# andompesta/nodeembedding-to-communityembedding

Hardware: AMD Instinct MI355X
Metric: SGNS pair-updates/sec at d=128, 1M-node graph (higher is better)
Workload: dtype f32

## Files before the change

### include/come.h

```cpp
#ifndef COME_H_
#define COME_H_

#include <stdint.h>

#ifdef __cplusplus
extern "C" {
#endif

#define COME_ABI_VERSION 5

enum {
    COME_OK = 0,
    COME_E_INVALID = -1,
    COME_E_HIP = -2,
    COME_E_UNSUPPORTED = -3
};

enum {
    COME_MODE_HOGWILD = 0,
    COME_MODE_SEQUENTIAL = 1
};

#define COME_TABLE_PACKED 0x100

#define COME_HOT_NONE 0x200

#define COME_DEFAULT_HOT_SHARE 5e-6
#define COME_DEFAULT_HOT_SHARE_WIDE 8e-7

int come_abi_version(void);

const char *come_source_sha256(void);
const char *come_last_error(void);

int come_init(int device);

void come_exp_table(float *out1000);

int come_fast_version(void);

int come_sgns_o2(float *node, float *ctx, int64_t V, int d, const int32_t *walks, int64_t P,
                 int L, const uint64_t *seeds, int window, int negative, const uint32_t *table,
                 uint64_t T, float lr, float alpha, int mode, void *stream);

int come_pack_table(const uint32_t *table, uint64_t T, void *packed, int32_t *status,
                    void *stream);

int come_sgns_o1(float *node, int64_t V, int d, const int32_t *edges, int64_t E,
                 const uint64_t *seeds, int negative, const uint32_t *table, uint64_t T, float lr,
                 int mode, void *stream);

int come_sgns_o2_loss(const float *node, const float *ctx, int64_t V, int d, const int32_t *walks,
                      int64_t P, int L, const uint64_t *seeds, int window, int negative,
                      const uint32_t *table, uint64_t T, int flags, double *walk_out,
                      double *loss_out, int64_t *pairs_out, void *stream);
int come_sgns_pairs_loss(const float *inp, const float *out, int64_t V, int d,
                         const int32_t *rows_in, const int32_t *rows_pos, const int32_t *rows_neg,
                         int64_t M, int negative, double *pair_out, double *loss_out,
                         int64_t *pairs_out, void *stream);

int come_community_grad(float *x, int64_t V, int d, const float *pi, const float *mu,
                        const float *inv_cov, int K, float beta, float lr, int iters,
                        void *stream);

int come_community_loss(const float *x, int64_t V, int d, const float *pi, const float *prec_chol,
                        const float *mu_prec, const float *log_norm, int K, float *row_out,
                        double *loss_out, void *stream);

int come_gmm_resp(const float *x, int64_t V, int d, const float *prec_chol, const float *mu_prec,
                  const float *log_norm, int K, float *resp_out, void *stream);

int come_gmm_estep(const float *x, int64_t V, int d, const float *prec_chol, const float *mu_prec,
                   const float *log_norm, int K, float *resp_out, float *lse_out, void *stream);

int come_gmm_scatter(const float *x, int64_t V, int d, const float *resp, const float *means,
                     int K, int chunks, float *scratch, float *scatter_out, void *stream);

int come_gmm_params(const double *scatter, const double *nk, const double *means,
                    const double *weights, int K, int d, double reg_covar, double *cov_out,
                    double *prec_chol_out, float *e_prec_chol, float *e_mu_prec,
                    float *e_log_norm, int *info, void *stream);

int come_gmm_estep_diag(const float *x, int64_t V, int d, const float *prec_sqrt,
                        const float *mu_prec, const float *log_norm, int K, float *resp_out,
                        float *lse_out, void *stream);
int come_gmm_diag_scratch(int64_t V, int d, int K, int cus, int *chunks_out,
                          int *rows_per_chunk_out);
int come_gmm_diag_moments(const float *x, int64_t V, int d, const float *resp, int K, int chunks,
                          void *scratch, double *nk_out, double *sx_out, void *stream);
int come_gmm_diag_scatter(const float *x, int64_t V, int d, const float *resp, const float *means,
                          int K, int chunks, void *scratch, double *ssq_out, void *stream);
int come_community_grad_diag(float *x, int64_t V, int d, const float *pi, const float *mu,
                             const float *inv_var, int K, float beta, float lr, int iters,
                             void *stream);
int come_community_loss_diag(const float *x, int64_t V, int d, const float *pi,
                             const float *prec_sqrt, const float *mu_prec, const float *log_norm,
                             int K, float *row_out, double *loss_out, void *stream);

int come_kmeans_scratch(int64_t V, int d, int K, int cus, int *chunks_out,
                        int *rows_per_chunk_out);
int come_kmeans_lloyd(const float *x, int64_t V, int d, const float *centers, int K, int chunks,
                      void *scratch, int32_t *labels_out, float *mindist_out, double *sums_out,
                      int64_t *counts_out, double *inertia_out, void *stream);
int come_kmeans_assign(const float *x, int64_t V, int d, const float *centers, int K,
                       int32_t *labels_out, float *mindist_out, void *stream);
int come_kmeans_update(float *centers, const double *sums, const int64_t *counts, int K, int d,
                       double *stats2, void *stream);

int come_kmeans_pp_scratch(int64_t V, int d, int T, int cus, int *chunks_out,
                           int *rows_per_chunk_out);
int come_kmeans_pp_step(const float *x, int64_t V, int d, const float *closest,
                        const int32_t *cand, int T, int chunks, float *dist_out, double *ppot,
                        double *pots_out, void *stream);
int come_kmeans_pp_pick(const float *dist, int64_t V, int T, const double *ppot,
                        const double *pots, int chunks, float *closest_out, double *cpot_out,
                        int32_t *best_out, double *pot_out, void *stream);
int come_kmeans_pp_sample(const float *closest, int64_t V, const double *cpot, int chunks,
                          int rows_per_chunk, const double *u, int T, int32_t *cand_out,
                          void *stream);


int come_random_walks(const int64_t *rowptr, const int32_t *col, int64_t V,
                      const int32_t *starts, int64_t P, int path_length, float alpha,
                      uint64_t seed, int64_t walk_offset, const int32_t *emit, int32_t *out,
                      void *stream);

int come_walks_reference(const int64_t *rowptr, const int32_t *col, int64_t V, int n_streams,
                         const int32_t *paths_per_stream, uint32_t *states, int path_length,
                         double alpha, const int32_t *emit, int threads, int32_t *out);

int come_pyrandom_seed(uint64_t seed, uint32_t *state625);

int come_pyrandom_draw(uint32_t *state625, int kind, uint64_t arg, int64_t count, double *out);

int come_np_draw_seeds(uint32_t *state625, int64_t n, uint64_t *out);

int come_graph_from_edges(const int64_t *edges, int64_t E, int64_t *node_ids, int64_t *V_out,
                          int64_t *rowptr, int32_t *col, int64_t *degree, int32_t *edge_pos,
                          int64_t *E_out);

int come_read_int_rows(const char *path, int64_t *rows, int64_t cap_rows, int width,
                       int64_t *nrows_out, int *max_tokens_out);
int come_write_int_rows(const char *path, const int64_t *rows, int64_t nrows, int width,
                        int append);
int come_save_embedding(const char *path, const float *emb, int64_t V, int d, int64_t first_id);
int come_format_f32(float x, char *out32);

int come_delta_begin(const float *W, const float *S, float *D, float *Down, int64_t n,
                     void *stream);
int come_delta_end(float *W, float *S, const float *Dsum, const float *Down, int64_t n,
                   void *stream);

int come_delta_flags(const float *W, const float *S, int64_t rows, int d, uint8_t *flags,
                     void *stream);
int come_delta_gather(const float *W, const float *S, const int64_t *idx, int64_t n, int d,
                      float *D, float *Down, void *stream);
int come_delta_scatter(float *W, float *S, const int64_t *idx, int64_t n, int d,
                       const float *Dsum, const float *Down, void *stream);

typedef struct come_launch_opts {
    int o2_kernel;
    int o2_blocks_per_cu;
    int o2_waves_per_block;
    int o2_static;
    int rows_per_wave;
    int o1_rows_per_wave;
    int max_waves;
    int o1_blocks_per_cu;
    int resident_cap;
    int community_async;
    int gmm_cov_async;
    int walk_staged;
    int o2_fresh_loads;
    int o2_atomic_writeback;
    int gmm_resp16;
    int o1_chunk;
    uint64_t *o2_update_count;
} come_launch_opts;

int come_get_options(come_launch_opts *out);

int come_set_option(const char *name, int value);

int come_sgns_o2_ex(float *node, float *ctx, int64_t V, int d, const int32_t *walks, int64_t P,
                    int L, const uint64_t *seeds, int window, int negative,
                    const uint32_t *table, uint64_t T, float lr, float alpha, int mode,
                    const uint32_t *hot_rows, const come_launch_opts *opts, void *stream);

int come_hot_rows(const uint32_t *table, uint64_t T, int64_t V, uint64_t min_count,
                  uint32_t *counts, uint32_t *hot_bits, void *stream);
int come_sgns_o1_ex(float *node, int64_t V, int d, const int32_t *edges, int64_t E,
                    const uint64_t *seeds, int negative, const uint32_t *table, uint64_t T,
                    float lr, int mode, const uint32_t *hot_rows, const come_launch_opts *opts,
                    void *stream);

int come_cpu_sgns_o2(float *node, float *ctx, int64_t V, int d, const int32_t *walks, int64_t P,
                     int L, const uint64_t *seeds, int window, int negative, const uint32_t *table,
                     uint64_t T, float lr, float alpha, int mode, int threads, int64_t *pairs_out);
int come_cpu_sgns_o1(float *node, int64_t V, int d, const int32_t *edges, int64_t E,
                     const uint64_t *seeds, int negative, const uint32_t *table, uint64_t T,
                     float lr, int mode, int threads, int64_t *pairs_out);
int come_cpu_community_grad(float *x, int64_t V, int d, const float *pi, const float *mu,
                            const float *inv_cov, int K, float beta, float lr, int iters,
                            int threads);
int come_cpu_gmm_resp(const float *x, int64_t V, int d, const float *prec_chol,
                      const float *mu_prec, const float *log_norm, int K, float *resp_out,
                      int threads);
int come_cpu_gmm_estep(const float *x, int64_t V, int d, const float *prec_chol,
                       const float *mu_prec, const float *log_norm, int K, float *resp_out,
                       float *lse_out, int threads);
int come_cpu_community_loss(const float *x, int64_t V, int d, const float *pi,
                            const float *prec_chol, const float *mu_prec, const float *log_norm,
                            int K, float *row_out, double *loss_out, int threads);
int come_cpu_sgns_o2_loss(const float *node, const float *ctx, int64_t V, int d,
                          const int32_t *walks, int64_t P, int L, const uint64_t *seeds,
                          int window, int negative, const uint32_t *table, uint64_t T,
                          double *walk_out, double *loss_out, int64_t *pairs_out, int threads);
int come_cpu_sgns_pairs_loss(const float *inp, const float *out, int64_t V, int d,
                             const int32_t *rows_in, const int32_t *rows_pos,
                             const int32_t *rows_neg, int64_t M, int negative, double *pair_out,
                             double *loss_out, int64_t *pairs_out, int threads);


int come_make_table(const double *counts_by_id, int64_t V, uint32_t *table, uint64_t T,
                    double power);

int come_lcg_table_draws(uint64_t seed, int64_t count, const uint32_t *table, uint64_t T,
                         uint32_t *out);

int64_t come_count_o2_pairs(const int32_t *walks, int64_t P, int L, int window);

#ifdef __cplusplus
}
#endif

#endif
```

### nodeembedding-to-communityembedding_amd/_lib.py

```python
import contextlib
import ctypes
import os

HERE = os.path.dirname(os.path.abspath(__file__))
DEFAULT_LIB_PATH = os.path.join(HERE, "libcome.so")
LIB_PATH = os.environ.get("COME_LIB_PATH") or DEFAULT_LIB_PATH

MODE_HOGWILD = 0
MODE_SEQUENTIAL = 1
TABLE_PACKED = 0x100
HOT_NONE = 0x200
ABI_VERSION = 5

SYMBOLS = ("come_abi_version", "come_last_error", "come_init", "come_exp_table",
           "come_fast_version", "come_sgns_o2", "come_sgns_o1", "come_community_grad",
           "come_gmm_resp", "come_make_table", "come_count_o2_pairs", "come_set_option",
           "come_random_walks", "come_walks_reference", "come_pyrandom_seed",
           "come_pyrandom_draw", "come_np_draw_seeds", "come_graph_from_edges",
           "come_read_int_rows",
           "come_write_int_rows", "come_save_embedding", "come_format_f32",
           "come_gmm_estep", "come_gmm_scatter", "come_gmm_params", "come_pack_table",
           "come_delta_begin", "come_delta_end", "come_get_options", "come_sgns_o2_ex",
           "come_sgns_o1_ex", "come_hot_rows", "come_lcg_table_draws", "come_delta_flags",
           "come_delta_gather", "come_delta_scatter", "come_cpu_sgns_o2", "come_cpu_sgns_o1",
           "come_cpu_community_grad", "come_cpu_gmm_resp", "come_cpu_gmm_estep",
           "come_source_sha256", "come_kmeans_scratch", "come_kmeans_lloyd",
           "come_kmeans_assign", "come_kmeans_update", "come_kmeans_pp_scratch",
           "come_kmeans_pp_step", "come_kmeans_pp_pick", "come_kmeans_pp_sample",
           "come_community_loss", "come_cpu_community_loss", "come_sgns_o2_loss",
           "come_sgns_pairs_loss", "come_cpu_sgns_o2_loss", "come_cpu_sgns_pairs_loss",
           "come_gmm_estep_diag", "come_gmm_diag_scratch", "come_gmm_diag_moments",
           "come_gmm_diag_scatter", "come_community_grad_diag", "come_community_loss_diag")

OPTION_FIELDS = ("o2_kernel", "o2_blocks_per_cu", "o2_waves_per_block",
                 "o2_static", "rows_per_wave", "o1_rows_per_wave",
                 "max_waves", "o1_blocks_per_cu", "resident_cap", "community_async",
                 "gmm_cov_async", "walk_staged", "o2_fresh_loads", "o2_atomic_writeback",
                 "gmm_resp16", "o1_chunk")


class LaunchOpts(ctypes.Structure):
    _fields_ = [(f, ctypes.c_int) for f in OPTION_FIELDS] + [("o2_update_count",
                                                             ctypes.c_void_p)]

_lib = None


def source_sha256():
    import hashlib
    csrc = os.path.join(HERE, "csrc")
    header = os.path.join(os.path.dirname(HERE), "include", "come.h")
    if not os.path.isdir(csrc) or not os.path.exists(header):
        return None
    names = sorted(f for f in os.listdir(csrc) if f.endswith((".hip", ".cpp", ".h")))
    h = hashlib.sha256()
    for f in [os.path.join(csrc, n) for n in names] + [os.path.join(csrc, "Makefile"), header]:
        with open(f, "rb") as fh:
            h.update(fh.read())
    return h.hexdigest()


class ComeError(RuntimeError):
    pass


def build():
    import subprocess
    subprocess.check_call(["make", "-s", "-C", os.path.join(HERE, "csrc"), "-j4"])


def lib():
    global _lib
    if _lib is not None:
        return _lib
    if not os.path.exists(LIB_PATH):
        raise ComeError("libcome.so not found at %s -- build it with "
                        "`make -C nodeembedding-to-communityembedding_amd/csrc` or "
                        "`python -c 'import __graft_entry__ as g; g.build()'`" % LIB_PATH)
    import torch
    L = ctypes.CDLL(LIB_PATH)
    P, i32, i64, u64, f32, f64 = (ctypes.c_void_p, ctypes.c_int, ctypes.c_int64, ctypes.c_uint64,
                                  ctypes.c_float, ctypes.c_double)
    L.come_abi_version.restype = i32
    L.come_source_sha256.restype = ctypes.c_char_p
    L.come_last_error.restype = ctypes.c_char_p
    L.come_init.argtypes = [i32]
    L.come_exp_table.argtypes = [P]
    L.come_exp_table.restype = None
    L.come_sgns_o2.argtypes = [P, P, i64, i32, P, i64, i32, P, i32, i32, P, u64, f32, f32, i32, P]
    L.come_sgns_o1.argtypes = [P, i64, i32, P, i64, P, i32, P, u64, f32, i32, P]
    L.come_community_grad.argtypes = [P, i64, i32, P, P, P, i32, f32, f32, i32, P]
    L.come_community_loss.argtypes = [P, i64, i32, P, P, P, P, i32, P, P, P]
    L.come_gmm_resp.argtypes = [P, i64, i32, P, P, P, i32, P, P]
    L.come_pack_table.argtypes = [P, u64, P, P, P]
    L.come_delta_begin.argtypes = [P, P, P, P, i64, P]
    L.come_delta_end.argtypes = [P, P, P, P, i64, P]
    L.come_gmm_estep.argtypes = [P, i64, i32, P, P, P, i32, P, P, P]
    L.come_gmm_scatter.argtypes = [P, i64, i32, P, P, i32, i32, P, P, P]
    L.come_gmm_params.argtypes = [P, P, P, P, i32, i32, f64, P, P, P, P, P, P, P]
    L.come_gmm_estep_diag.argtypes = [P, i64, i32, P, P, P, i32, P, P, P]
    L.come_gmm_diag_scratch.argtypes = [i64, i32, i32, i32, P, P]
    L.come_gmm_diag_moments.argtypes = [P, i64, i32, P, i32, i32, P, P, P, P]
    L.come_gmm_diag_scatter.argtypes = [P, i64, i32, P, P, i32, i32, P, P, P]
    L.come_community_grad_diag.argtypes = [P, i64, i32, P, P, P, i32, f32, f32, i32, P]
    L.come_community_loss_diag.argtypes = [P, i64, i32, P, P, P, P, i32, P, P, P]
    L.come_kmeans_scratch.argtypes = [i64, i32, i32, i32, P, P]
    L.come_kmeans_lloyd.argtypes = [P, i64, i32, P, i32, i32, P, P, P, P, P, P, P]
    L.come_kmeans_assign.argtypes = [P, i64, i32, P, i32, P, P, P]
    L.come_kmeans_update.argtypes = [P, P, P, i32, i32, P, P]
    L.come_kmeans_pp_scratch.argtypes = [i64, i32, i32, i32, P, P]
    L.come_kmeans_pp_step.argtypes = [P, i64, i32, P, P, i32, i32, P, P, P, P]
    L.come_kmeans_pp_pick.argtypes = [P, i64, i32, P, P, i32, P, P, P, P, P]
    L.come_kmeans_pp_sample.argtypes = [P, i64, P, i32, i32, P, i32, P, P]
    L.come_make_table.argtypes = [P, i64, P, u64, f64]
    L.come_count_o2_pairs.argtypes = [P, i64, i32, i32]
    L.come_count_o2_pairs.restype = i64
    L.come_set_option.argtypes = [ctypes.c_char_p, i32]
    L.come_get_options.argtypes = [P]
    L.come_sgns_o2_ex.argtypes = [P, P, i64, i32, P, i64, i32, P, i32, i32, P, u64, f32, f32, i32,
                                  P, P, P]
    L.come_hot_rows.argtypes = [P, u64, i64, u64, P, P, P]
    L.come_lcg_table_draws.argtypes = [u64, i64, P, u64, P]
    L.come_delta_flags.argtypes = [P, P, i64, i32, P, P]
    L.come_delta_gather.argtypes = [P, P, P, i64, i32, P, P, P]
    L.come_delta_scatter.argtypes = [P, P, P, i64, i32, P, P, P]
    L.come_sgns_o1_ex.argtypes = [P, i64, i32, P, i64, P, i32, P, u64, f32, i32, P, P, P]
    L.come_cpu_sgns_o2.argtypes = [P, P, i64, i32, P, i64, i32, P, i32, i32, P, u64, f32, f32,
                                   i32, i32, P]
    L.come_cpu_sgns_o1.argtypes = [P, i64, i32, P, i64, P, i32, P, u64, f32, i32, i32, P]
    L.come_cpu_community_grad.argtypes = [P, i64, i32, P, P, P, i32, f32, f32, i32, i32]
    L.come_cpu_gmm_resp.argtypes = [P, i64, i32, P, P, P, i32, P, i32]
    L.come_cpu_gmm_estep.argtypes = [P, i64, i32, P, P, P, i32, P, P, i32]
    L.come_cpu_community_loss.argtypes = [P, i64, i32, P, P, P, P, i32, P, P, i32]
    L.come_sgns_o2_loss.argtypes = [P, P, i64, i32, P, i64, i32, P, i32, i32, P, u64, i32, P, P, P,
                                    P]
    L.come_sgns_pairs_loss.argtypes = [P, P, i64, i32, P, P, P, i64, i32, P, P, P, P]
    L.come_cpu_sgns_o2_loss.argtypes = [P, P, i64, i32, P, i64, i32, P, i32, i32, P, u64, P, P, P,
                                        i32]
    L.come_cpu_sgns_pairs_loss.argtypes = [P, P, i64, i32, P, P, P, i64, i32, P, P, P, i32]
    cp = ctypes.c_char_p
    L.come_random_walks.argtypes = [P, P, i64, P, i64, i32, f32, u64, i64, P, P, P]
    L.come_walks_reference.argtypes = [P, P, i64, i32, P, P, i32, f64, P, i32, P]
    L.come_pyrandom_seed.argtypes = [u64, P]
    L.come_pyrandom_draw.argtypes = [P, i32, u64, i64, P]
    L.come_np_draw_seeds.argtypes = [P, i64, P]
    L.come_graph_from_edges.argtypes = [P, i64, P, P, P, P, P, P, P]
    L.come_read_int_rows.argtypes = [cp, P, i64, i32, P, P]
    L.come_write_int_rows.argtypes = [cp, P, i64, i32, i32]
    L.come_save_embedding.argtypes = [cp, P, i64, i32, i64]
    L.come_format_f32.argtypes = [f32, cp]
    if L.come_abi_version() != ABI_VERSION:
        raise ComeError("libcome.so ABI version %d, this binding needs %d (rebuild the library)"
                        % (L.come_abi_version(), ABI_VERSION))
    want = source_sha256()
    if want is not None and LIB_PATH == DEFAULT_LIB_PATH:
        got = L.come_source_sha256().decode()
        if got != want:
            raise ComeError("%s was built from other sources (stamp %s, the sources beside it "
                            "hash to %s): rebuild it with `make -C %s`" % (
                                LIB_PATH, got[:12], want[:12], os.path.join(HERE, "csrc")))
    _lib = L
    return L


def check(rc, what):
    if rc != 0:
        msg = lib().come_last_error().decode(errors="replace")
        raise ComeError("%s failed (rc=%d): %s" % (what, rc, msg))


def ptr(t):
    if hasattr(t, "data_ptr"):
        return ctypes.c_void_p(t.data_ptr())
    return t.ctypes.data_as(ctypes.c_void_p)


def stream_handle(device=None):
    import torch
    return ctypes.c_void_p(torch.cuda.current_stream(device).cuda_stream)


def set_option(name, value):
    check(lib().come_set_option(name.encode(), int(value)), "come_set_option(%s)" % name)


def launch_opts(update_count=None, **overrides):
    o = LaunchOpts()
    check(lib().come_get_options(ctypes.byref(o)), "come_get_options")
    for k, v in overrides.items():
        if k not in OPTION_FIELDS:
            raise ValueError("unknown launch option %r" % k)
        setattr(o, k, int(v))
    if update_count is not None:
        o.o2_update_count = update_count.data_ptr()
    return o


@contextlib.contextmanager
def options(**kv):
    cur = launch_opts()
    old = {k: getattr(cur, k) for k in kv}
    try:
        for k, v in kv.items():
            set_option(k, v)
        yield
    finally:
        for k, v in old.items():
            set_option(k, v)
```

### nodeembedding-to-communityembedding_amd/context_embeddings.py

```python
import logging as log
import time

import numpy as np

from . import training_sdg_inner as tsi
from .embedding import walks_to_rows

DEFAULT_SYNC_WALKS = 1 << 19


def o2_pairs(rows, window):
    import torch
    if isinstance(rows, torch.Tensor):
        lens = (rows >= 0).sum(dim=1).long()
        return int(torch.where(lens >= window + 1, 2 * window * lens - window * (window + 1),
                               lens * (lens - 1)).sum())
    return tsi.count_o2_pairs(rows, window)


class Context2Vec(object):
    def __init__(self, lr=0.1, window_size=5, workers=1, negative=5, deterministic=False,
                 batch_walks=1 << 20, distributed=False, sync_walks=DEFAULT_SYNC_WALKS,
                 sparse_sync=False, overlap=True, group=None, hot_share=None, launch_opts=None,
                 combine="touched_mean"):
        self.lr = float(lr)
        self.workers = workers
        self.negative = negative
        self.window_size = int(window_size)
        self.deterministic = deterministic
        self.batch_walks = int(batch_walks)
        self.distributed = bool(distributed)
        self.sync_walks = int(sync_walks)
        self.sparse_sync = bool(sparse_sync)
        self.overlap = bool(overlap)
        self.group = group
        self.hot_share = hot_share
        self.launch_opts = launch_opts
        self.combine = combine
        self._exchanges = {}
        if self.distributed and self.deterministic:
            raise ValueError("distributed=True trains Hogwild shards; deterministic=True is the "
                             "one-wavefront parity mode")

    def world(self):
        from .distributed import world_of
        return world_of(self.group) if self.distributed else (0, 1)

    def exchange(self, model):
        from .distributed import DeltaAllReduce, SparseDeltaAllReduce
        key = (id(model.node_embedding), id(model.context_embedding))
        ex = self._exchanges.get(key)
        if ex is None:
            cls = SparseDeltaAllReduce if self.sparse_sync else DeltaAllReduce
            self._exchanges = {key: cls([model.node_embedding, model.context_embedding],
                                        group=self.group, combine=self.combine)}
            return self._exchanges[key]
        ex.reset()
        return ex

    def loss(self, model, paths, alpha=1.0, seeds=None, mean=False, return_pairs=False):
        import torch
        rows = walks_to_rows(model, paths, max_len=tsi.MAX_SENTENCE_LEN)
        P = rows.shape[0]
        if seeds is None:
            ab = np.random.RandomState(0).randint(0, 2 ** 24, size=2 * P).astype(np.uint64)
            seeds = (ab[0::2] << np.uint64(24)) + ab[1::2]
        elif not isinstance(seeds, torch.Tensor):
            seeds = np.ascontiguousarray(seeds, np.uint64)
        if seeds.shape != (P,):
            raise ValueError("seeds must hold one value per walk (%d)" % P)
        rank, world = self.world()
        if world > 1:
            from .distributed import shard_walks
            rows, seeds = shard_walks(rows, seeds, rank, world)
        dev = model.node_embedding.device
        table = model.negative_table() if self.negative > 0 else None
        total, pairs = 0.0, 0
        for b in range(0, rows.shape[0], self.batch_walks):
            w = rows[b:b + self.batch_walks]
            w = w.contiguous() if isinstance(w, torch.Tensor) else \
                torch.from_numpy(np.ascontiguousarray(w, np.int32)).to(dev)
            sd = seeds[b:b + self.batch_walks]
            sd = sd.contiguous() if isinstance(sd, torch.Tensor) else \
                torch.from_numpy(np.ascontiguousarray(sd, np.uint64).view(np.int64)).to(dev)
            t, p = tsi.sgns_o2_loss(model.node_embedding, model.context_embedding, w, sd,
                                    self.window_size, self.negative, table)
            total += t
            pairs += p
        if world > 1:
            from .distributed import all_reduce_sum
            tt = torch.tensor([total], dtype=torch.float64, device=dev)
            pp = torch.tensor([pairs], dtype=torch.int64, device=dev)
            all_reduce_sum([tt], self.group)
            all_reduce_sum([pp], self.group)
            total, pairs = float(tt[0]), int(pp[0])
        value = alpha * total
        if mean:
            value = value / pairs if pairs else 0.0
        return (value, pairs) if return_pairs else value

    def train(self, model, paths, total_nodes, alpha=1.0, node_count=0, chunksize=150):
        import torch
        assert model.node_embedding.dtype == torch.float32
        assert model.context_embedding.dtype == torch.float32
        if alpha <= 0.:
            return 0
        if total_nodes is None:
            raise AttributeError('need the number of node')
        start = time.time()
        rows = walks_to_rows(model, paths, max_len=tsi.MAX_SENTENCE_LEN)
        seeds = tsi.draw_seeds(rows.shape[0])
        rank, world = self.world()
        n_batches = None
        if world > 1:
            from .distributed import shard_range, shard_walks
            lo, hi = shard_range(rows.shape[0], 0, world)
            n_batches = max(1, -(-(hi - lo) // self.sync_walks))
            rows, seeds = shard_walks(rows, seeds, rank, world)
        pairs = o2_pairs(rows, self.window_size)
        n_valid = int((rows >= 0).sum())
        self.train_rows(model, rows, seeds, alpha, n_batches=n_batches)
        if model.node_embedding.is_cuda:
            torch.cuda.synchronize(model.node_embedding.device)
        elapsed = time.time() - start
        nodes = n_valid + node_count
        log.info("O2 training on %i nodes (%i pair updates%s) took %.2fs, %.0f pairs/s",
                 nodes, pairs, " on rank %d of %d" % (rank, world) if world > 1 else "",
                 elapsed, pairs / elapsed if elapsed else 0.0)
        return pairs

    def train_rows(self, model, rows, seeds, alpha=1.0, n_batches=None, update_count=None,
                   launch_events=None):
        import torch
        dev = model.node_embedding.device
        mode = tsi.MODE_SEQUENTIAL if self.deterministic else tsi.MODE_HOGWILD
        hot = None if self.deterministic else model.hot_rows(self.hot_share)
        table = model.negative_table()
        rank, world = self.world()
        ex = self.exchange(model) if world > 1 else None
        P = rows.shape[0]
        if ex is None:
            batch = self.batch_walks
            n_batches = -(-P // batch)
        else:
            batch = self.sync_walks
            n_batches = n_batches if n_batches is not None else max(1, -(-P // batch))
        stream = torch.cuda.current_stream(dev) if launch_events is not None else None
        for b in range(n_batches):
            w = rows[b * batch:(b + 1) * batch]
            if w.shape[0]:
                w = w.contiguous() if isinstance(w, torch.Tensor) else \
                    torch.from_numpy(np.ascontiguousarray(w, np.int32)).to(dev)
                sd = seeds[b * batch:(b + 1) * batch]
                sd = sd if isinstance(sd, torch.Tensor) else \
                    torch.from_numpy(np.ascontiguousarray(sd, np.uint64).view(np.int64)).to(dev)
                if launch_events is not None:
                    ev = (torch.cuda.Event(enable_timing=True),
                          torch.cuda.Event(enable_timing=True))
                    ev[0].record(stream)
                tsi.sgns_o2(model.node_embedding, model.context_embedding, w, sd,
                            self.window_size, self.negative, table, self.lr, alpha, mode,
                            opts=self.launch_opts, hot=hot, update_count=update_count)
                if launch_events is not None:
                    ev[1].record(stream)
                    launch_events.append(ev)
            if ex is not None:
                if b + 1 < n_batches and self.overlap and getattr(ex, "overlap_safe", True):
                    ex.start()
                else:
                    ex.sync()
```

### nodeembedding-to-communityembedding_amd/csrc/come_hot.hip

```cpp
#include "come_internal.h"

namespace come {

__global__ void __launch_bounds__(256) k_table_counts(const uint32_t *__restrict__ table,
                                                      uint64_t T, int64_t V,
                                                      uint32_t *__restrict__ counts) {
    const uint64_t n = (uint64_t)gridDim.x * blockDim.x;
    const int lane = threadIdx.x & 63;
    for (uint64_t base = (uint64_t)blockIdx.x * blockDim.x + (threadIdx.x & ~63u); base < T;
         base += n) {
        const uint64_t s = base + lane;
        const bool in = s < T;
        const uint32_t v = in ? table[s] : 0xFFFFFFFFu;
        const uint32_t first = (uint32_t)__shfl((int)v, 0);
        const bool uniform_wave = __all(!in || v == first) && first < (uint64_t)V;
        if (uniform_wave) {
            const int cnt = __popcll(__ballot(in));
            if (lane == 0) atomicAdd(counts + first, (uint32_t)cnt);
        } else if (in && (int64_t)v < V) {
            atomicAdd(counts + v, 1u);
        }
    }
}

__global__ void __launch_bounds__(256) k_table_counts_packed(const uint4 *__restrict__ words,
                                                             uint64_t T, int64_t V,
                                                             uint32_t *__restrict__ counts) {
    const uint64_t n = (uint64_t)gridDim.x * blockDim.x;
    const int lane = threadIdx.x & 63;
    for (uint64_t base = (uint64_t)blockIdx.x * blockDim.x + (threadIdx.x & ~63u); base < T;
         base += n) {
        const uint64_t s = base + lane;
        const bool in = s < T;
        const uint4 wd = words[base >> 6];
        const uint64_t bits = ((uint64_t)wd.w << 32) | wd.z;
        const uint64_t mask = lane == 63 ? ~0ull : ((2ull << lane) - 1ull);
        const uint32_t v = in ? wd.x + (uint32_t)__popcll(bits & mask) : 0xFFFFFFFFu;
        const uint32_t first = (uint32_t)__shfl((int)v, 0);
        const bool uniform_wave = __all(!in || v == first) && first < (uint64_t)V;
        if (uniform_wave) {
            const int cnt = __popcll(__ballot(in));
            if (lane == 0) atomicAdd(counts + first, (uint32_t)cnt);
        } else if (in && (int64_t)v < V) {
            atomicAdd(counts + v, 1u);
        }
    }
}

__global__ void __launch_bounds__(256) k_hot_bits(const uint32_t *__restrict__ counts, int64_t V,
                                                  uint64_t min_count,
                                                  uint32_t *__restrict__ hot_bits) {
    const int64_t words = (V + 31) / 32;
    for (int64_t w = (int64_t)blockIdx.x * blockDim.x + threadIdx.x; w < words;
         w += (int64_t)gridDim.x * blockDim.x) {
        uint32_t bits = 0;
        for (int b = 0; b < 32; ++b) {
            const int64_t r = 32 * w + b;
            if (r < V && counts[r] >= min_count) bits |= 1u << b;
        }
        hot_bits[w] = bits;
    }
}

static int hot_rows_impl(int dev, const uint32_t *table, uint64_t T, int packed, int64_t V,
                         uint64_t min_count, uint32_t *counts, uint32_t *hot_bits, void *stream) {
    hipError_t e = hipMemsetAsync(counts, 0, sizeof(uint32_t) * (size_t)V, (hipStream_t)stream);
    if (e != hipSuccess) return hip_error(e, "hipMemsetAsync(counts)");
    uint64_t blocks = (T + 255) / 256;
    const uint64_t cap = (uint64_t)num_cus(dev) * 16;
    if (blocks > cap) blocks = cap;
    if (packed)
        hipLaunchKernelGGL(k_table_counts_packed, dim3((unsigned)blocks), dim3(256), 0,
                           (hipStream_t)stream, (const uint4 *)table, T, V, counts);
    else
        hipLaunchKernelGGL(k_table_counts, dim3((unsigned)blocks), dim3(256), 0,
                           (hipStream_t)stream, table, T, V, counts);
    int rc = hip_error(hipGetLastError(), "k_table_counts launch");
    if (rc) return rc;
    const int64_t words = (V + 31) / 32;
    int64_t wb = (words + 255) / 256;
    if (wb > 4096) wb = 4096;
    hipLaunchKernelGGL(k_hot_bits, dim3((unsigned)wb), dim3(256), 0, (hipStream_t)stream,
                       (const uint32_t *)counts, V, min_count, hot_bits);
    return hip_error(hipGetLastError(), "k_hot_bits launch");
}

int derive_hot_rows(int dev, const uint32_t *table, uint64_t T, int packed, int64_t V, int d,
                    void *stream, const uint32_t **bits_out) {
    uint32_t *counts = (uint32_t *)stream_scratch(dev, stream, kScratchHotCounts,
                                                  sizeof(uint32_t) * (size_t)V);
    uint32_t *bits = (uint32_t *)stream_scratch(dev, stream, kScratchHotBits,
                                                sizeof(uint32_t) * (size_t)((V + 31) / 32));
    if (!counts || !bits) return scratch_failed();
    const double share = d <= 128 ? COME_DEFAULT_HOT_SHARE : COME_DEFAULT_HOT_SHARE_WIDE;
    uint64_t min_count = (uint64_t)(share * (double)T);
    if (min_count < 1) min_count = 1;
    *bits_out = bits;
    return hot_rows_impl(dev, table, T, packed, V, min_count, counts, bits, stream);
}

}

using namespace come;

extern "C" int come_hot_rows(const uint32_t *table, uint64_t T, int64_t V, uint64_t min_count,
                             uint32_t *counts, uint32_t *hot_bits, void *stream) {
    if (V <= 0 || V > INT32_MAX) return set_error(COME_E_INVALID, "hot_rows: V out of range");
    if (!table || !counts || !hot_bits || T == 0)
        return set_error(COME_E_INVALID, "hot_rows: null pointer or empty table");
    int dev = 0;
    int rc = ensure_init(&dev);
    if (rc) return rc;
    return hot_rows_impl(dev, table, T, 0, V, min_count, counts, hot_bits, stream);
}
```

### nodeembedding-to-communityembedding_amd/csrc/come_sgns.hip

```cpp
#include <string.h>

#include <map>
#include <mutex>
#include <tuple>

#include "come_sgns_impl.h"

namespace come {

constexpr size_t kRingMaxWaveBytes = 40 * 1024;
constexpr int64_t kStreamRowsPerWave = 32;

static int64_t hog_max_blocks(const come_launch_opts &o, int64_t V, int wpb, int rows_per_wave) {
    int64_t waves = 0;
    if (rows_per_wave > 0) waves = V / rows_per_wave > 1 ? V / rows_per_wave : 1;
    if (o.max_waves > 0 && (waves == 0 || o.max_waves < waves)) waves = o.max_waves;
    return waves > 0 ? (waves + wpb - 1) / wpb : 0;
}

static const KernelSet &kernel_set(int d, int *full) {
    const int vec = d <= 64 ? 1 : d <= 128 ? 2 : d <= 256 ? 4 : 8;
    *full = (vec > 1 && d == 64 * vec) ? 1 : 0;
    switch (vec) {
        case 1: return kernels_vec1();
        case 2: return kernels_vec2();
        case 4: return kernels_vec4();
        default: return kernels_vec8();
    }
}
static int maxn_index(int n) { return n <= 5 ? 0 : (n <= 10 ? 1 : 2); }

static int resident_blocks(void *fn, int threads, size_t lds) {
    static std::mutex mu;
    static std::map<std::tuple<void *, int, size_t>, int> cache;
    std::lock_guard<std::mutex> lock(mu);
    const auto key = std::make_tuple(fn, threads, lds);
    auto it = cache.find(key);
    if (it != cache.end()) return it->second;
    int n = 0;
    if (hipOccupancyMaxActiveBlocksPerMultiprocessor(&n, (const void *)fn, threads, lds) !=
            hipSuccess || n < 0) {
        (void)hipGetLastError();
        n = 0;
    }
    cache[key] = n;
    return n;
}

static int launch(const come_launch_opts &o, void *fn, void *args, int64_t units, int mode,
                  int wpb, int blocks_per_cu, size_t lds_bytes, void *stream,
                  int64_t max_blocks = 0) {
    int dev = 0;
    int rc = ensure_init(&dev);
    if (rc) return rc;
    dim3 grid, block;
    if (mode == COME_MODE_SEQUENTIAL) {
        grid = dim3(1);
        block = dim3(64);
    } else {
        int64_t blocks = (units + wpb - 1) / wpb;
        const int res = resident_blocks(fn, 64 * wpb, lds_bytes);
        if (res > 0 && blocks_per_cu > res && o.resident_cap) blocks_per_cu = res;
        int64_t cap = (int64_t)num_cus(dev) * blocks_per_cu;
        if (max_blocks > 0 && max_blocks < cap) cap = max_blocks;
        if (blocks > cap) blocks = cap;
        grid = dim3((unsigned)(blocks > 0 ? blocks : 1));
        block = dim3(64 * wpb);
    }
    void *kargs[] = {args};
    hipError_t e = hipLaunchKernel(fn, grid, block, kargs, lds_bytes, (hipStream_t)stream);
    return hip_error(e, "kernel launch");
}

}

using namespace come;

static int check_common(int64_t V, int d, int negative, const uint32_t *table, uint64_t T,
                        int &mode, int &packed, int &hot_none) {
    packed = (mode & COME_TABLE_PACKED) ? 1 : 0;
    hot_none = (mode & COME_HOT_NONE) ? 1 : 0;
    mode &= ~(COME_TABLE_PACKED | COME_HOT_NONE);
    if (packed && ((uintptr_t)table % 16) != 0)
        return set_error(COME_E_INVALID, "packed table must be 16-byte aligned");
    if (V <= 0) return set_error(COME_E_INVALID, "V must be > 0 (got %lld)", (long long)V);
    if (V > INT32_MAX)
        return set_error(COME_E_INVALID, "V must fit int32 row indices (got %lld)", (long long)V);
    if (d < 1 || d > kMaxDim)
        return set_error(COME_E_INVALID, "d must be in [1, %d] (got %d)", kMaxDim, d);
    if (negative < 0 || negative > kMaxNegative)
        return set_error(COME_E_INVALID, "negative must be in [0, %d] (got %d)", kMaxNegative,
                         negative);
    if (negative > 0 && (table == nullptr || T == 0))
        return set_error(COME_E_INVALID, "negative sampling needs a non-empty table");
    if (mode != COME_MODE_HOGWILD && mode != COME_MODE_SEQUENTIAL)
        return set_error(COME_E_INVALID, "mode must be COME_MODE_HOGWILD or COME_MODE_SEQUENTIAL");
    return COME_OK;
}

static bool aligned_for(const void *p, int d) {
    const int vec = (d + 63) / 64;
    if (d != 64 * vec || vec < 2) return true;
    const int bytes = (vec >= 4 ? 16 : 8);
    return ((uintptr_t)p % bytes) == 0;
}

extern "C" int come_sgns_o2_ex(float *node, float *ctx, int64_t V, int d, const int32_t *walks,
                               int64_t P, int L, const uint64_t *seeds, int window, int negative,
                               const uint32_t *table, uint64_t T, float lr, float alpha, int mode,
                               const uint32_t *hot_rows, const come_launch_opts *opts,
                               void *stream) {
    const come_launch_opts o = opts ? *opts : current_opts();
    int packed = 0, hot_none = 0;
    int rc = check_common(V, d, negative, table, T, mode, packed, hot_none);
    if (rc) return rc;
    if (P < 0 || L < 0 || window < 0)
        return set_error(COME_E_INVALID, "P, L and window must be >= 0");
    if (mode == COME_MODE_HOGWILD && o.o2_kernel == 2)
        return set_error(COME_E_INVALID, "o2_kernel=2 (LDS ring) is the sequential kernel only");
    if (P == 0 || L == 0) return COME_OK;
    if (!node || !ctx || !walks || !seeds)
        return set_error(COME_E_INVALID, "null node/ctx/walks/seeds pointer");
    if (!aligned_for(node, d) || !aligned_for(ctx, d))
        return set_error(COME_E_INVALID, "node/ctx must be 16-byte aligned for d=%d", d);
    if (hot_none) {
        hot_rows = nullptr;
    } else if (mode == COME_MODE_HOGWILD && hot_rows == nullptr && table != nullptr && T > 0) {
        int dev = 0;
        rc = ensure_init(&dev);
        if (rc) return rc;
        rc = derive_hot_rows(dev, table, T, packed, V, d, stream, &hot_rows);
        if (rc) return rc;
    }
    O2Args a{node, ctx, walks, seeds, table, V, P, L, d, window, negative, lr, alpha,
             make_fastmod(T), packed, nullptr,
             reinterpret_cast<unsigned long long *>(o.o2_update_count), o.o2_fresh_loads,
             o.o2_atomic_writeback, mode == COME_MODE_HOGWILD ? hot_rows : nullptr};
    int full = 0;
    const KernelSet &ks = kernel_set(d, &full);
    const int mi = maxn_index(negative);
    const bool hog = mode == COME_MODE_HOGWILD;
    const int wpb = (o.max_waves > 0 && o.max_waves < 4) ? o.max_waves : 4;
    if (hog && (o.o2_kernel == 0 || o.o2_kernel == 3) && window <= 31) {
        int dev = 0;
        rc = ensure_init(&dev);
        if (rc) return rc;
        const int bpc = o.o2_blocks_per_cu > 0 ? o.o2_blocks_per_cu : 8;
        const int64_t hcap = hog_max_blocks(o, V, wpb, o.rows_per_wave);
        int64_t blocks = (P + wpb - 1) / wpb;
        if (blocks > (int64_t)num_cus(dev) * bpc) blocks = (int64_t)num_cus(dev) * bpc;
        if (hcap > 0 && blocks > hcap) blocks = hcap;
        if (o.o2_kernel == 3 || V >= kStreamRowsPerWave * wpb * blocks) {
            if (!o.o2_static) a.counter = launch_counter(dev, stream);
            return launch(o, ks.o2_stream[full][mi], &a, P, mode, wpb, bpc, 0, stream, hcap);
        }
    }
    const int rs = 2 * window + 1;
    const size_t wave_bytes = 4 * (size_t)((rs * d + 3) & ~3);
    const bool ring_ok = rs <= 64 && wave_bytes <= kRingMaxWaveBytes;
    if (!hog && o.o2_kernel != 1 && ring_ok)
        return launch(o, ks.o2_ring[full][mi], &a, P, mode, 1, 1, wave_bytes, stream);
    return launch(o, ks.o2_direct[full][mi], &a, P, mode, wpb,
                  o.o2_blocks_per_cu > 0 ? o.o2_blocks_per_cu : 6, 0, stream,
                  hog ? hog_max_blocks(o, V, wpb, o.rows_per_wave) : 0);
}

extern "C" int come_sgns_o2(float *node, float *ctx, int64_t V, int d, const int32_t *walks,
                            int64_t P, int L, const uint64_t *seeds, int window, int negative,
                            const uint32_t *table, uint64_t T, float lr, float alpha, int mode,
                            void *stream) {
    return come_sgns_o2_ex(node, ctx, V, d, walks, P, L, seeds, window, negative, table, T, lr,
                           alpha, mode, nullptr, nullptr, stream);
}

extern "C" int come_sgns_o1_ex(float *node, int64_t V, int d, const int32_t *edges, int64_t E,
                               const uint64_t *seeds, int negative, const uint32_t *table,
                               uint64_t T, float lr, int mode, const uint32_t *hot_rows,
                               const come_launch_opts *opts, void *stream) {
    const come_launch_opts o = opts ? *opts : current_opts();
    int packed = 0, hot_none = 0;
    int rc = check_common(V, d, negative, table, T, mode, packed, hot_none);
    if (rc) return rc;
    if (E < 0) return set_error(COME_E_INVALID, "E must be >= 0");
    if (E == 0) return COME_OK;
    if (!node || !edges || !seeds) return set_error(COME_E_INVALID, "null node/edges/seeds");
    if (2 * negative > 64)
        return set_error(COME_E_INVALID, "O1 supports negative <= 32 (got %d)", negative);
    if (!aligned_for(node, d))
        return set_error(COME_E_INVALID, "node must be 16-byte aligned for d=%d", d);
    if (hot_none) {
        hot_rows = nullptr;
    } else if (mode == COME_MODE_HOGWILD && hot_rows == nullptr && table != nullptr && T > 0) {
        int dev = 0;
        rc = ensure_init(&dev);
        if (rc) return rc;
        rc = derive_hot_rows(dev, table, T, packed, V, d, stream, &hot_rows);
        if (rc) return rc;
    }
    const int bpc = o.o1_blocks_per_cu > 0 ? o.o1_blocks_per_cu
                    : (o.o1_chunk != 0 && d <= 128 && negative <= 5) ? 8 : 6;
    const int64_t hcap = mode == COME_MODE_HOGWILD ? hog_max_blocks(o, V, 4, o.o1_rows_per_wave) : 0;
    int64_t chunk = o.o1_chunk;
    if (chunk < 0) {
        int dev = 0;
        rc = ensure_init(&dev);
        if (rc) return rc;
        int64_t blocks = (int64_t)num_cus(dev) * bpc;
        if (hcap > 0 && hcap < blocks) blocks = hcap;
        const int64_t waves = mode == COME_MODE_HOGWILD ? 4 * blocks : 1;
        chunk = (E + waves - 1) / waves;
    }
    O1Args a{node,           edges, seeds, table, V, E, d, negative, lr, make_fastmod(T), packed,
             mode == COME_MODE_HOGWILD ? hot_rows : nullptr, chunk > 0 ? chunk : 1};
    int full = 0;
    const KernelSet &ks = kernel_set(d, &full);
    if (chunk > 0)
        return launch(o, ks.o1_runs[full][maxn_index(negative)], &a, (E + chunk - 1) / chunk, mode,
                      4, bpc, 0, stream, hcap);
    return launch(o, ks.o1[full][maxn_index(negative)], &a, E, mode, 4,
                  o.o1_blocks_per_cu > 0 ? o.o1_blocks_per_cu : 6, 0, stream,
                  mode == COME_MODE_HOGWILD ? hog_max_blocks(o, V, 4, o.o1_rows_per_wave) : 0);
}

extern "C" int come_sgns_o1(float *node, int64_t V, int d, const int32_t *edges, int64_t E,
                            const uint64_t *seeds, int negative, const uint32_t *table, uint64_t T,
                            float lr, int mode, void *stream) {
    return come_sgns_o1_ex(node, V, d, edges, E, seeds, negative, table, T, lr, mode, nullptr,
                           nullptr, stream);
}

__global__ void __launch_bounds__(256) k_pack_table(const uint32_t *__restrict__ table, uint64_t T,
                                                    uint4 *__restrict__ packed,
                                                    int32_t *__restrict__ status) {
    const int lane = threadIdx.x & 63;
    const uint64_t words = (T + 63) / 64;
    const uint64_t nwaves = (uint64_t)gridDim.x * (blockDim.x >> 6);
    bool bad = false;
    for (uint64_t w = (uint64_t)blockIdx.x * (blockDim.x >> 6) + (threadIdx.x >> 6); w < words;
         w += nwaves) {
        const uint64_t s = w * 64 + lane;
        const uint32_t v = s < T ? table[s] : 0u;
        const uint32_t prev = (uint32_t)__shfl_up((int)v, 1);
        const uint32_t step = v - prev;
        const bool inc = lane > 0 && s < T && step == 1u;
        bad |= lane > 0 && s < T && step > 1u;
        const uint64_t bits = __ballot(inc);
        if (lane == 0) packed[w] = make_uint4(v, 0u, (uint32_t)bits, (uint32_t)(bits >> 32));
    }
    if (__any(bad) && lane == 0) atomicOr(status, 1);
}

extern "C" int come_pack_table(const uint32_t *table, uint64_t T, void *packed, int32_t *status,
                               void *stream) {
    if (!table || !packed || !status || T == 0)
        return set_error(COME_E_INVALID, "pack_table: null pointer or empty table");
    if (((uintptr_t)packed % 16) != 0)
        return set_error(COME_E_INVALID, "packed table must be 16-byte aligned");
    int dev = 0;
    int rc = ensure_init(&dev);
    if (rc) return rc;
    hipError_t e = hipMemsetAsync(status, 0, sizeof(int32_t), (hipStream_t)stream);
    if (e != hipSuccess) return hip_error(e, "hipMemsetAsync(status)");
    const uint64_t words = (T + 63) / 64;
    uint64_t blocks = (words + 3) / 4;
    const uint64_t cap = (uint64_t)num_cus(dev) * 8;
    if (blocks > cap) blocks = cap;
    hipLaunchKernelGGL(k_pack_table, dim3((unsigned)blocks), dim3(256), 0, (hipStream_t)stream,
                       table, T, (uint4 *)packed, status);
    return hip_error(hipGetLastError(), "k_pack_table launch");
}

extern "C" int come_upload_exp_table(const float *host1000) {
    hipError_t (*const up[])(const float *) = {upload_exp_table_vec1, upload_exp_table_vec2,
                                                upload_exp_table_vec4, upload_exp_table_vec8};
    for (auto f : up) {
        const int rc = hip_error(f(host1000), "hipMemcpyToSymbol(exp table)");
        if (rc) return rc;
    }
    return COME_OK;
}
```

### nodeembedding-to-communityembedding_amd/csrc/come_sgns_impl.h

```cpp
#pragma once
#include <hip/hip_runtime.h>
#include <stdint.h>

#include "come_internal.h"
#include "come_wave.h"

namespace come {

static __constant__ float c_exp_table[kExpTableSize];

struct LcgLane {
    uint64_t a, c;
};

__device__ inline LcgLane lcg_lane_constants(int k) {
    uint64_t a = 1, c = 0;
    for (int i = 0; i < k; ++i) {
        a = (a * kLcgMul) & kLcgMask;
        c = (c * kLcgMul + kLcgAdd) & kLcgMask;
    }
    return {a, c};
}

__device__ inline uint64_t lcg_next(uint64_t s) { return (s * kLcgMul + kLcgAdd) & kLcgMask; }

struct LcgTable {
    uint64_t a[64], c[64];
};
constexpr LcgTable make_lcg_table() {
    LcgTable t{};
    uint64_t a = 1, c = 0;
    for (int k = 0; k < 64; ++k) {
        t.a[k] = a;
        t.c[k] = c;
        a = (a * kLcgMul) & kLcgMask;
        c = (c * kLcgMul + kLcgAdd) & kLcgMask;
    }
    return t;
}
static __constant__ LcgTable c_lcg = make_lcg_table();
constexpr LcgTable kLcgHost = make_lcg_table();
constexpr uint64_t kLcgA64 = (kLcgHost.a[63] * kLcgMul) & kLcgMask;
constexpr uint64_t kLcgC64 = (kLcgHost.c[63] * kLcgMul + kLcgAdd) & kLcgMask;

struct LcgFromTable {
    int lane;
};
__device__ inline uint64_t lcg_state_of(uint64_t base, const LcgLane &lc) {
    return (lc.a * base + lc.c) & kLcgMask;
}
__device__ inline uint64_t lcg_state_of(uint64_t base, const LcgFromTable &lt) {
    return (c_lcg.a[lt.lane] * base + c_lcg.c[lt.lane]) & kLcgMask;
}

__device__ inline uint32_t table_slot(uint64_t s, uint64_t m, uint32_t d) {
    const uint32_t x = (uint32_t)(s >> 16);
    if (d == 0) return x;
    return (uint32_t)__umul64hi(m * (uint64_t)x, (uint64_t)d);
}

struct PackedWord {
    uint32_t base;
    uint32_t unused;
    uint64_t bits;
};

template <class Args>
__device__ inline uint32_t table_value(const Args &a, uint32_t slot) {
    if (a.packed) {
        const uint4 w = reinterpret_cast<const uint4 *>(a.table)[slot >> 6];
        const uint64_t bits = ((uint64_t)w.w << 32) | w.z;
        const uint64_t mask = (2ull << (slot & 63)) - 1ull;
        return w.x + (uint32_t)__popcll(bits & mask);
    }
    return a.table[slot];
}

__device__ inline int uniform(int v) { return __builtin_amdgcn_readfirstlane(v); }
__device__ inline float uniformf(float v) {
    return __int_as_float(__builtin_amdgcn_readfirstlane(__float_as_int(v)));
}
__device__ inline uint64_t uniform64(uint64_t v) {
    const uint32_t lo = __builtin_amdgcn_readfirstlane((uint32_t)v);
    const uint32_t hi = __builtin_amdgcn_readfirstlane((uint32_t)(v >> 32));
    return ((uint64_t)hi << 32) | lo;
}
__device__ inline uint32_t readlane_u32(uint32_t v, int lane) {
    return (uint32_t)__builtin_amdgcn_readlane((int)v, lane);
}
__device__ inline uint64_t readlane_u64(uint64_t v, int lane) {
    const uint32_t lo = readlane_u32((uint32_t)v, lane);
    const uint32_t hi = readlane_u32((uint32_t)(v >> 32), lane);
    return ((uint64_t)hi << 32) | lo;
}

template <int VEC, bool FULL>
struct Row {
    float v[VEC];

    __device__ inline void load(const float *__restrict__ row, int lane, int d) {
#pragma unroll
        for (int i = 0; i < VEC; ++i) {
            const int e = lane + 64 * i;
            v[i] = (FULL || e < d) ? row[e] : 0.0f;
        }
    }

    __device__ inline void load_nt(const float *__restrict__ row, int lane, int d) {
#pragma unroll
        for (int i = 0; i < VEC; ++i) {
            const int e = lane + 64 * i;
            v[i] = (FULL || e < d) ? __builtin_nontemporal_load(row + e) : 0.0f;
        }
    }

    __device__ inline void load_fresh(const float *__restrict__ row, int lane, int d) {
#pragma unroll
        for (int i = 0; i < VEC; ++i) {
            const int e = lane + 64 * i;
            v[i] = (FULL || e < d) ? __hip_atomic_load(row + e, __ATOMIC_RELAXED,
                                                       __HIP_MEMORY_SCOPE_AGENT)
                                   : 0.0f;
        }
    }

    __device__ inline void load_as(const float *__restrict__ row, int lane, int d, bool fresh) {
        if (fresh) load_fresh(row, lane, d);
        else load(row, lane, d);
    }

    __device__ inline void store(float *__restrict__ row, int lane, int d) const {
#pragma unroll
        for (int i = 0; i < VEC; ++i) {
            const int e = lane + 64 * i;
            if (FULL || e < d) row[e] = v[i];
        }
    }

    __device__ inline void atomic_add(float *__restrict__ row, int lane, int d) const {
#pragma unroll
        for (int i = 0; i < VEC; ++i) {
            const int e = lane + 64 * i;
            if (FULL || e < d) atomicAdd(row + e, v[i]);
        }
    }
};

template <int VEC, bool FULL>
__device__ inline float lane_partial(const Row<VEC, FULL> &a, const Row<VEC, FULL> &b) {
    float p = 0.0f;
#pragma unroll
    for (int i = 0; i < VEC; ++i) p = __builtin_fmaf(a.v[i], b.v[i], p);
    return p;
}

__device__ inline float wave_sum(float p) {
    p = reduce_stage<0>(p);
    p = reduce_stage<1>(p);
    p = reduce_stage<2>(p);
    p = reduce_stage<3>(p);
    p = reduce_stage<4>(p);
    return reduce_stage<5>(p);
}

template <int N>
__device__ inline void wave_sum_n(float (&part)[N], int count) {
#define COME_STAGE(S)                                          \
    _Pragma("unroll") for (int k = 0; k < N; ++k) if (k < count) part[k] = reduce_stage<S>(part[k]);
    COME_STAGE(0) COME_STAGE(1) COME_STAGE(2) COME_STAGE(3) COME_STAGE(4) COME_STAGE(5)
#undef COME_STAGE
}

template <int N>
__device__ inline void wave_sum_all(float (&part)[N]) {
#define COME_STAGE(S) \
    _Pragma("unroll") for (int k = 0; k < N; ++k) part[k] = reduce_stage<S>(part[k]);
    COME_STAGE(0) COME_STAGE(1) COME_STAGE(2) COME_STAGE(3) COME_STAGE(4) COME_STAGE(5)
#undef COME_STAGE
}

__device__ inline bool sigmoid_ref(float f, float *sig) {
    if (f <= -(float)kMaxExp || f >= (float)kMaxExp) return false;
    const int b = (int)(((double)f + 6.0) * 83.0);
    *sig = c_exp_table[b];
    return true;
}

__device__ inline bool sigmoid_tab(const float *tab, float f, float *sig) {
    if (f <= -(float)kMaxExp || f >= (float)kMaxExp) return false;
    const int b = (int)(((double)f + 6.0) * 83.0);
    *sig = tab[b];
    return true;
}

struct DrawBatch {
    uint32_t target;
    uint64_t base;
    int used;
};

template <class Args>
__device__ inline void draws_fill(DrawBatch &b, uint64_t state0, const LcgLane &lc,
                                  const Args &a, int count = 64) {
    b.base = state0;
    b.used = 0;
    b.target = 0;
    if ((int)(threadIdx.x & 63) < count) {
        const uint64_t s = (lc.a * state0 + lc.c) & kLcgMask;
        b.target = table_value(a, table_slot(s, a.fm.m, a.fm.d));
    }
}

__device__ inline uint64_t draws_state_at_used(const DrawBatch &b, const LcgLane &lc) {
    const uint64_t s = (lc.a * b.base + lc.c) & kLcgMask;
    if (b.used < 64) return uniform64(readlane_u64(s, b.used));
    return lcg_next(uniform64(readlane_u64(s, 63)));
}

struct DrawPipe {
    uint32_t t0, t1;
    uint64_t base0, base1;
    int used;

    template <class Args, class Lcg>
    __device__ inline uint32_t gather(uint64_t base, const Lcg &lc, const Args &a) {
        const uint64_t s = lcg_state_of(base, lc);
        return table_value(a, table_slot(s, a.fm.m, a.fm.d));
    }

    template <class Args, class Lcg>
    __device__ inline uint32_t gather_hot(uint64_t base, const Lcg &lc, const Args &a) {
        const uint32_t v = gather(base, lc, a);
        if (a.hot == nullptr || (int64_t)v >= a.V) return v;
        return v | (((a.hot[v >> 5] >> (v & 31)) & 1u) << 31);
    }
};


struct O2Args {
    float *node;
    float *ctx;
    const int32_t *walks;
    const uint64_t *seeds;
    const uint32_t *table;
    int64_t V;
    int64_t P;
    int L;
    int d;
    int window;
    int negative;
    float lr;
    float alpha;
    FastMod fm;
    int packed;
    int64_t *counter;
    unsigned long long *upd_count;
    int fresh;
    int wb_atomic;
    const uint32_t *hot;
};

template <class Args>
__device__ inline bool is_hot(const Args &a, int r) {
    return a.hot != nullptr && ((a.hot[(uint32_t)r >> 5] >> (r & 31)) & 1u);
}

__device__ inline int64_t next_unit(int64_t *counter, int64_t cur, int64_t stride, int lane) {
    if (!counter) return cur + stride;
    int64_t v = 0;
    if (lane == 0) v = (int64_t)atomicAdd((unsigned long long *)counter, 1ull);
    return (int64_t)uniform64((uint64_t)v);
}

__device__ inline uint64_t advance64_uniform(uint64_t base) {
    return (kLcgA64 * base + kLcgC64) & kLcgMask;
}
__device__ inline uint64_t advance64(uint64_t base, const LcgLane &lc) {
    const uint64_t s = (lc.a * base + lc.c) & kLcgMask;
    return lcg_next(uniform64(readlane_u64(s, 63)));
}

template <int VEC, bool FULL>
__device__ inline void atomic_add_delta(float *__restrict__ row, const Row<VEC, FULL> &cur,
                                        const Row<VEC, FULL> &orig, int lane, int d) {
    Row<VEC, FULL> delta;
#pragma unroll
    for (int e = 0; e < VEC; ++e) delta.v[e] = cur.v[e] - orig.v[e];
    delta.atomic_add(row, lane, d);
}

template <int VEC, bool FULL, int MAXN>
__device__ inline void o2_pair(const O2Args &a, DrawBatch &db, const LcgLane &lc, int lane, int ci,
                               Row<VEC, FULL> &pos, bool &pos_upd, Row<VEC, FULL> &in,
                               Row<VEC, FULL> &work, int &nupd) {
    using R = Row<VEC, FULL>;
    const int n = a.negative;
    const int d = a.d;
    if (n > 0 && db.used + n > 64) draws_fill(db, draws_state_at_used(db, lc), lc, a);
    int t[MAXN + 1];
    bool valid[MAXN + 1];
    t[0] = ci;
    valid[0] = true;
#pragma unroll
    for (int k = 1; k <= MAXN; ++k) {
        if (k <= n) {
            const int tk = (int)readlane_u32(db.target, db.used + k - 1);
            t[k] = tk;
            valid[k] = tk != ci && tk >= 0 && tk < a.V;
        } else {
            t[k] = -1;
            valid[k] = false;
        }
    }
    if (n > 0) db.used += n;

    R r[MAXN + 1], o[MAXN + 1];
#pragma unroll
    for (int k = 1; k <= MAXN; ++k)
        if (valid[k]) {
            r[k].load_as(a.ctx + (int64_t)t[k] * d, lane, d, a.fresh);
            o[k] = r[k];
        }

    float part[MAXN + 1];
    part[0] = lane_partial(in, pos);
#pragma unroll
    for (int k = 1; k <= MAXN; ++k) part[k] = valid[k] ? lane_partial(in, r[k]) : 0.0f;
    wave_sum_n(part, n + 1);

#pragma unroll
    for (int e = 0; e < VEC; ++e) work.v[e] = 0.0f;
    {
        float sig;
        if (sigmoid_ref(uniformf(part[0]), &sig)) {
            const float g = ((1.0f - sig) * a.lr) * a.alpha;
#pragma unroll
            for (int e = 0; e < VEC; ++e) {
                work.v[e] = __builtin_fmaf(g, pos.v[e], work.v[e]);
                pos.v[e] = __builtin_fmaf(g, in.v[e], pos.v[e]);
            }
            pos_upd = true;
            ++nupd;
        }
    }
    bool upd[MAXN + 1];
    upd[0] = false;
#pragma unroll
    for (int k = 1; k <= MAXN; ++k) {
        upd[k] = false;
        if (!valid[k]) continue;
        float f = part[k];
        int prev = -1;
#pragma unroll
        for (int q = 1; q < k; ++q)
            if (valid[q] && t[q] == t[k]) prev = q;
        if (prev >= 0) {
#pragma unroll
            for (int q = 1; q < k; ++q) {
                if (q == prev) {
                    r[k] = r[q];
                    f = upd[q] ? wave_sum(lane_partial(in, r[k])) : part[q];
                }
            }
        }
        f = uniformf(f);
        part[k] = f;
        float sig;
        if (!sigmoid_ref(f, &sig)) continue;
        const float g = ((0.0f - sig) * a.lr) * a.alpha;
#pragma unroll
        for (int e = 0; e < VEC; ++e) {
            work.v[e] = __builtin_fmaf(g, r[k].v[e], work.v[e]);
            r[k].v[e] = __builtin_fmaf(g, in.v[e], r[k].v[e]);
        }
        upd[k] = true;
        ++nupd;
    }
#pragma unroll
    for (int k = 1; k <= MAXN; ++k) {
        if (!upd[k]) continue;
        if (!a.wb_atomic && !is_hot(a, t[k])) {
            r[k].store(a.ctx + (int64_t)t[k] * d, lane, d);
            continue;
        }
        bool last = true;
#pragma unroll
        for (int q = k + 1; q <= MAXN; ++q)
            if (upd[q] && t[q] == t[k]) last = false;
        if (last) atomic_add_delta(a.ctx + (int64_t)t[k] * d, r[k], o[k], lane, d);
    }
#pragma unroll
    for (int e = 0; e < VEC; ++e) in.v[e] = in.v[e] + work.v[e];
}

template <int VEC, bool FULL, int MAXN>
__global__ void __launch_bounds__(256) k_sgns_o2(O2Args a) {
    using R = Row<VEC, FULL>;
    const int lane = threadIdx.x & 63;
    const int64_t waves_per_block = blockDim.x >> 6;
    const int64_t gw = (int64_t)blockIdx.x * waves_per_block + (threadIdx.x >> 6);
    const int64_t nwaves = (int64_t)gridDim.x * waves_per_block;
    const LcgLane lc = lcg_lane_constants(lane);
    const int d = a.d;
    const int path_len = a.L < kMaxSentenceLen ? a.L : kMaxSentenceLen;

    for (int64_t p = gw; p < a.P; p += nwaves) {
        const int32_t *__restrict__ idx = a.walks + p * (int64_t)a.L;
        DrawBatch db;
        db.used = 0;
        db.base = uniform64(a.seeds[p]);
        db.target = 0;
        if (a.negative > 0) draws_fill(db, db.base, lc, a);
        int nupd = 0;
        for (int i = 0; i < path_len; ++i) {
            const int ci = uniform(idx[i]);
            if (ci < 0 || ci >= a.V) continue;
            const int j0 = i - a.window < 0 ? 0 : i - a.window;
            const int j1 = i + a.window + 1 > path_len ? path_len : i + a.window + 1;
            for (int j = j0; j < j1; ++j) {
                if (j == i) continue;
                const int cj = uniform(idx[j]);
                if (cj < 0 || cj >= a.V) continue;
                R in, pos;
                in.load_as(a.node + (int64_t)cj * d, lane, d, a.fresh);
                pos.load_as(a.ctx + (int64_t)ci * d, lane, d, a.fresh);
                const R pos0 = pos;
                bool pos_upd = false;
                R work;
                o2_pair<VEC, FULL, MAXN>(a, db, lc, lane, ci, pos, pos_upd, in, work, nupd);
                if (pos_upd) {
                    if (a.wb_atomic || is_hot(a, ci))
                        atomic_add_delta(a.ctx + (int64_t)ci * d, pos, pos0, lane, d);
                    else
                        pos.store(a.ctx + (int64_t)ci * d, lane, d);
                }
                if (a.wb_atomic || is_hot(a, cj)) work.atomic_add(a.node + (int64_t)cj * d, lane, d);
                else in.store(a.node + (int64_t)cj * d, lane, d);
            }
        }
        if (a.upd_count && lane == 0 && nupd) atomicAdd(a.upd_count, (unsigned long long)nupd);
    }
}

template <int VEC, bool FULL, int MAXN>
__global__ void __launch_bounds__(128) k_sgns_o2_ring(O2Args a) {
    using R = Row<VEC, FULL>;
    extern __shared__ __attribute__((aligned(16))) float lds[];
    const int lane = threadIdx.x & 63;
    const int wib = threadIdx.x >> 6;
    const int64_t waves_per_block = blockDim.x >> 6;
    const int64_t gw = (int64_t)blockIdx.x * waves_per_block + wib;
    const int64_t nwaves = (int64_t)gridDim.x * waves_per_block;
    const LcgLane lc = lcg_lane_constants(lane);
    const int d = a.d;
    const int w = a.window;
    const int n = a.negative;
    const int RS = 2 * w + 1;
    const int path_len = a.L < kMaxSentenceLen ? a.L : kMaxSentenceLen;
    const int wave_floats = (RS * d + 3) & ~3;
    float *ring = lds + wib * wave_floats;
    auto valid_row = [&](int r) { return r >= 0 && r < a.V; };
    auto slot_add = [&](int s, int delta) {
        s += delta;
        if (s < 0) s += RS;
        if (s >= RS) s -= RS;
        return s;
    };

    for (int64_t p = a.counter ? next_unit(a.counter, 0, 0, lane) : gw; p < a.P;
         p = next_unit(a.counter, p, nwaves, lane)) {
        const int32_t *__restrict__ walk = a.walks + p * (int64_t)a.L;
        int wbase = 0;
        int c0 = lane < path_len ? walk[lane] : -1;
        int c1 = 64 + lane < path_len ? walk[64 + lane] : -1;
        auto idx_at = [&](int q) {
            if (q >= path_len) return -1;
            const int off = q - wbase;
            const int r = off < 64 ? __builtin_amdgcn_readlane(c0, off)
                                   : __builtin_amdgcn_readlane(c1, off - 64);
            return valid_row(r) ? r : -1;
        };
        DrawPipe dp;
        dp.used = 0;
        dp.base0 = uniform64(a.seeds[p]);
        dp.t0 = dp.t1 = 0;
        if (n > 0) {
            dp.t0 = dp.gather(dp.base0, lc, a);
            dp.base1 = advance64(dp.base0, lc);
            dp.t1 = dp.gather(dp.base1, lc, a);
        }
        auto take = [&](int k) -> int {
            const int q = dp.used + k;
            return (int)(q < 64 ? readlane_u32(dp.t0, q) : readlane_u32(dp.t1, q - 64));
        };
        auto advance = [&]() {
            if (n == 0) return;
            dp.used += n;
            if (dp.used >= 64) {
                dp.used -= 64;
                dp.t0 = dp.t1;
                dp.base0 = dp.base1;
                dp.base1 = advance64(dp.base1, lc);
                dp.t1 = dp.gather(dp.base1, lc, a);
            }
        };
        int tn[MAXN + 1];
        R rn[MAXN + 1];
        auto fetch_next = [&]() {
#pragma unroll
            for (int k = 1; k <= MAXN; ++k) {
                const int tk = k <= n ? take(k - 1) : -1;
                tn[k] = tk;
                rn[k].load(a.ctx + (int64_t)(valid_row(tk) ? tk : 0) * d, lane, d);
            }
        };
        fetch_next();

        int nupd = 0;
        int ids = -1;
        auto id_of = [&](int s) { return __builtin_amdgcn_readlane(ids, s); };
        auto alias_mask = [&](int id, int except) -> uint64_t {
            return __ballot(lane < RS && lane != except && ids == id);
        };
        auto set_id = [&](int s, int id) { ids = lane == s ? id : ids; };
        auto write_back = [&](int s, int id) {
            if (alias_mask(id, s) != 0) return;
            R row;
            row.load(ring + s * d, lane, d);
            row.store(a.node + (int64_t)id * d, lane, d);
        };
        auto enter_row = [&](int s, int id, const R &fetched) {
            const uint64_t m = alias_mask(id, s);
            if (m) {
                R row;
                row.load(ring + __builtin_ctzll(m) * d, lane, d);
                row.store(ring + s * d, lane, d);
            } else {
                fetched.store(ring + s * d, lane, d);
            }
            set_id(s, id);
        };
        for (int q = 0; q < w && q < path_len; ++q) {
            const int id = idx_at(q);
            if (id >= 0) {
                R row;
                row.load(a.node + (int64_t)id * d, lane, d);
                enter_row(q, id, row);
            }
        }
        R pos_n, ent_n;
        int pos_n_id = idx_at(0), ent_n_id = idx_at(w);
        pos_n.load(a.ctx + (int64_t)(pos_n_id >= 0 ? pos_n_id : 0) * d, lane, d);
        ent_n.load(a.node + (int64_t)(ent_n_id >= 0 ? ent_n_id : 0) * d, lane, d);

        int si = 0;
        for (int i = 0; i < path_len; ++i) {
            if (i + 1 + w >= wbase + 128) {
                wbase += 64;
                c0 = c1;
                c1 = wbase + 64 + lane < path_len ? walk[wbase + 64 + lane] : -1;
            }
            const int ci = pos_n_id;
            R pos = pos_n;
            const int se = slot_add(si, w);
            if (i + w < path_len || i - w - 1 >= 0) {
                const int old_id = i - w - 1 >= 0 ? id_of(se) : -1;
                if (old_id >= 0 && old_id == ent_n_id) {
                } else {
                    if (old_id >= 0) write_back(se, old_id);
                    set_id(se, -1);
                    if (i + w < path_len && ent_n_id >= 0) enter_row(se, ent_n_id, ent_n);
                }
            }
            pos_n_id = idx_at(i + 1);
            ent_n_id = idx_at(i + 1 + w);
            pos_n.load(a.ctx + (int64_t)(pos_n_id >= 0 ? pos_n_id : 0) * d, lane, d);
            ent_n.load(a.node + (int64_t)(ent_n_id >= 0 ? ent_n_id : 0) * d, lane, d);

            if (ci >= 0) {
                bool pos_upd = false;
                const int j0 = i - w < 0 ? 0 : i - w;
                const int j1 = i + w + 1 > path_len ? path_len : i + w + 1;
                for (int j = j0; j < j1; ++j) {
                    if (j == i) continue;
                    const int sj = slot_add(si, j - i);
                    const int cj = id_of(sj);
                    if (cj < 0) continue;
                    R in;
                    in.load(ring + sj * d, lane, d);
                    int t[MAXN + 1];
                    R r[MAXN + 1];
#pragma unroll
                    for (int k = 1; k <= MAXN; ++k) {
                        t[k] = tn[k];
                        r[k] = rn[k];
                    }
                    advance();
                    fetch_next();

                    bool valid[MAXN + 1];
#pragma unroll
                    for (int k = 1; k <= MAXN; ++k)
                        valid[k] = k <= n && t[k] != ci && valid_row(t[k]);
                    float part[MAXN + 1];
                    part[0] = lane_partial(in, pos);
#pragma unroll
                    for (int k = 1; k <= MAXN; ++k) part[k] = lane_partial(in, r[k]);
                    wave_sum_n(part, n + 1);
                    R work;
#pragma unroll
                    for (int e = 0; e < VEC; ++e) work.v[e] = 0.0f;
                    {
                        float sig;
                        if (sigmoid_ref(uniformf(part[0]), &sig)) {
                            const float g = ((1.0f - sig) * a.lr) * a.alpha;
#pragma unroll
                            for (int e = 0; e < VEC; ++e) {
                                work.v[e] = __builtin_fmaf(g, pos.v[e], work.v[e]);
                                pos.v[e] = __builtin_fmaf(g, in.v[e], pos.v[e]);
                            }
                            pos_upd = true;
                            ++nupd;
                        }
                    }
                    bool upd[MAXN + 1];
#pragma unroll
                    for (int k = 1; k <= MAXN; ++k) {
                        upd[k] = false;
                        if (!valid[k]) continue;
                        float f = part[k];
                        int prev = -1;
#pragma unroll
                        for (int q = 1; q < k; ++q)
                            if (valid[q] && t[q] == t[k]) prev = q;
                        if (prev >= 0) {
#pragma unroll
                            for (int q = 1; q < k; ++q) {
                                if (q == prev) {
                                    r[k] = r[q];
                                    f = upd[q] ? wave_sum(lane_partial(in, r[k])) : part[q];
                                }
                            }
                        }
                        f = uniformf(f);
                        part[k] = f;
                        float sig;
                        if (!sigmoid_ref(f, &sig)) continue;
                        const float g = ((0.0f - sig) * a.lr) * a.alpha;
#pragma unroll
                        for (int e = 0; e < VEC; ++e) {
                            work.v[e] = __builtin_fmaf(g, r[k].v[e], work.v[e]);
                            r[k].v[e] = __builtin_fmaf(g, in.v[e], r[k].v[e]);
                        }
                        upd[k] = true;
                        ++nupd;
                    }
#pragma unroll
                    for (int k = 1; k <= MAXN; ++k) {
                        if (!upd[k]) continue;
                        r[k].store(a.ctx + (int64_t)t[k] * d, lane, d);
#pragma unroll
                        for (int q = 1; q <= MAXN; ++q)
                            if (tn[q] == t[k]) rn[q] = r[k];
                        if (pos_n_id == t[k]) pos_n = r[k];
                    }
#pragma unroll
                    for (int e = 0; e < VEC; ++e) in.v[e] = in.v[e] + work.v[e];
                    uint64_t m = alias_mask(cj, -1);
                    while (m) {
                        const int rr = __builtin_ctzll(m);
                        m &= m - 1;
                        in.store(ring + rr * d, lane, d);
                    }
                }
                if (pos_upd) {
                    pos.store(a.ctx + (int64_t)ci * d, lane, d);
#pragma unroll
                    for (int q = 1; q <= MAXN; ++q)
                        if (tn[q] == ci) rn[q] = pos;
                    if (pos_n_id == ci) pos_n = pos;
                }
            }
            si = slot_add(si, 1);
        }
        const int first = path_len - w - 1 > 0 ? path_len - w - 1 : 0;
        for (int q = first; q < path_len; ++q) {
            const int s = q % RS;
            const int id = id_of(s);
            if (id >= 0) write_back(s, id);
            set_id(s, -1);
        }
        if (a.upd_count && lane == 0 && nupd) atomicAdd(a.upd_count, (unsigned long long)nupd);
    }
}

template <int VEC, int MAXN>
constexpr int stream_waves_per_eu() {
    return (VEC <= 2 && MAXN <= 5) ? 8 : 1;
}

template <int VEC, bool FULL, int MAXN>
__global__ void __launch_bounds__(256)
    __attribute__((amdgpu_waves_per_eu(stream_waves_per_eu<VEC, MAXN>())))
    k_sgns_o2_stream(O2Args a) {
    using R = Row<VEC, FULL>;
    const int lane = threadIdx.x & 63;
    const int64_t waves_per_block = blockDim.x >> 6;
    const int64_t gw = (int64_t)blockIdx.x * waves_per_block + (threadIdx.x >> 6);
    const int64_t nwaves = (int64_t)gridDim.x * waves_per_block;
    const LcgFromTable lc{lane};
    const int d = a.d;
    const int w = a.window;
    const int n = a.negative;
    const int path_len = a.L < kMaxSentenceLen ? a.L : kMaxSentenceLen;
    const uint32_t Vu = (uint32_t)a.V;
    auto valid_row = [&](int r) { return (uint32_t)r < Vu; };
    constexpr bool kReread = VEC <= 2;
    constexpr uint32_t kHotBit = 0x80000000u;
    constexpr int kWaitVm0 = 0x0F70;
    __shared__ float s_exp[kExpTableSize];
    for (int i = threadIdx.x; i < kExpTableSize; i += blockDim.x) s_exp[i] = c_exp_table[i];
    __syncthreads();
    __shared__ uint32_t s_draws[4][128];
    uint32_t *draws = s_draws[threadIdx.x >> 6];
    __shared__ int s_walk[4][128];
    int *wpos = s_walk[threadIdx.x >> 6];

    for (int64_t p = a.counter ? next_unit(a.counter, 0, 0, lane) : gw; p < a.P;
         p = next_unit(a.counter, p, nwaves, lane)) {
        const int32_t *__restrict__ walk = a.walks + p * (int64_t)a.L;
        auto chunk = [&](int q0) {
            const int q = q0 + lane;
            int v = q < path_len ? walk[q] : -1;
            if (!valid_row(v)) return -1;
            if (a.hot != nullptr && ((a.hot[(uint32_t)v >> 5] >> (v & 31)) & 1u))
                v = (int)((uint32_t)v | kHotBit);
            return v;
        };
        int wbase = 0;
        wpos[lane] = chunk(0);
        wpos[64 + lane] = chunk(64);
        __builtin_amdgcn_wave_barrier();
        auto raw_at = [&](int q) {
            if (q >= path_len) return -1;
            while (q - wbase >= 128) {
                wbase += 64;
                wpos[lane] = wpos[64 + lane];
                wpos[64 + lane] = chunk(wbase + 64);
                __builtin_amdgcn_wave_barrier();
            }
            return uniform(wpos[q - wbase]);
        };
        int it_i = 0, it_j = -1;
        auto next_pair = [&](int &ci, int &cj, int &pi, bool &hi, bool &hj) -> bool {
            for (;;) {
                if (it_i >= path_len) return false;
                const int i = it_i;
                const int j0 = i - w < 0 ? 0 : i - w;
                const int j1 = i + w + 1 > path_len ? path_len : i + w + 1;
                if (it_j < j0) it_j = j0;
                const int rci = raw_at(i);
                if (rci == -1 || it_j >= j1) {
                    ++it_i;
                    it_j = -1;
                    continue;
                }
                const int j = it_j++;
                if (j == i) continue;
                const int rcj = raw_at(j);
                if (rcj == -1) continue;
                ci = (int)((uint32_t)rci & ~kHotBit);
                cj = (int)((uint32_t)rcj & ~kHotBit);
                hi = ((uint32_t)rci & kHotBit) != 0;
                hj = ((uint32_t)rcj & kHotBit) != 0;
                pi = i;
                return true;
            }
        };
        DrawPipe dp;
        dp.used = 0;
        dp.base0 = uniform64(a.seeds[p]);
        if (n > 0) {
            draws[lane] = dp.gather_hot(dp.base0, lc, a);
            dp.base1 = advance64_uniform(dp.base0);
            draws[64 + lane] = dp.gather_hot(dp.base1, lc, a);
            __builtin_amdgcn_wave_barrier();
        }
        auto advance = [&]() {
            if (n == 0) return;
            dp.used += n;
            if (dp.used >= 64) {
                dp.used -= 64;
                draws[lane] = draws[64 + lane];
                dp.base0 = dp.base1;
                dp.base1 = advance64_uniform(dp.base1);
                draws[64 + lane] = dp.gather_hot(dp.base1, lc, a);
                __builtin_amdgcn_wave_barrier();
            }
        };
        int nci = -1, ncj = -1, npi = -1;
        bool nhi = false, nhj = false;
        R in_n, pos_n, rn[MAXN + 1];
        R padd;
        bool padd_on = false;
        int prev_i = -1;
        static_assert(MAXN < 32, "the alias test keeps a pair's rows in half a wavefront");
        uint32_t ids = 0xFFFFFFFFu;
        auto next_target = [&](int k) {
            return k <= n ? (int)(readlane_u32(ids, 32 + k) & ~kHotBit) : -1;
        };
        auto prefetch = [&](bool need_pos) {
            in_n.load(a.node + (int64_t)ncj * d, lane, d);
            if (need_pos) pos_n.load(a.ctx + (int64_t)nci * d, lane, d);
            const bool drawn = lane > 32 && lane <= 32 + n;
            const uint32_t nx = drawn ? draws[drawn ? dp.used + lane - 33 : 0] : 0xFFFFFFFFu;
            ids = lane < 32 ? ids : lane == 32 ? (uint32_t)nci : nx;
#pragma unroll
            for (int k = 1; k <= MAXN; ++k) {
                const int tk = next_target(k);
                rn[k].load_nt(a.ctx + (int64_t)(valid_row(tk) ? tk : 0) * d, lane, d);
            }
        };
        auto reread = [&](bool need_pos) {
            in_n.load_fresh(a.node + (int64_t)ncj * d, lane, d);
            if (need_pos) pos_n.load_fresh(a.ctx + (int64_t)nci * d, lane, d);
#pragma unroll
            for (int k = 1; k <= MAXN; ++k) {
                const int tk = next_target(k);
                rn[k].load_fresh(a.ctx + (int64_t)(valid_row(tk) ? tk : 0) * d, lane, d);
            }
        };
        bool have = next_pair(nci, ncj, npi, nhi, nhj);
        if (have) prefetch(true);
        if (kReread) __builtin_amdgcn_s_waitcnt(kWaitVm0);
        int nupd = 0;
        R pos;
        bool pos_upd = false;

        while (have) {
            const int ci = nci, cj = ncj, ic = npi;
            const bool hot_ci = nhi, hot_cj = nhj;
            R in = in_n;
            int t[MAXN + 1];
            R r[MAXN + 1];
#pragma unroll
            for (int k = 1; k <= MAXN; ++k) {
                t[k] = next_target(k);
                r[k] = rn[k];
            }
            const bool new_center = ic != prev_i;
            if (new_center || hot_ci) {
                pos = pos_n;
                if (kReread && padd_on)
#pragma unroll
                    for (int e = 0; e < VEC; ++e) pos.v[e] += padd.v[e];
            }
            if (new_center) pos_upd = false;
            prev_i = ic;
            ids = (uint32_t)__builtin_amdgcn_permlane32_swap((int)ids, (int)ids, false, false)[1];
            const uint32_t thm = (uint32_t)__ballot((ids & kHotBit) != 0);
            advance();
            have = next_pair(nci, ncj, npi, nhi, nhj);
            if (have) prefetch(npi != ic || nhi);

            const uint32_t idv = ids & ~kHotBit;
            uint64_t alias = __ballot(idv == (uint32_t)ci) & ~(1ull | (1ull << 32));
#pragma unroll
            for (int k = 1; k <= MAXN; ++k)
                alias |= __ballot(idv == (uint32_t)t[k]) & ~(1ull << k);
            const uint64_t negs = (2ull << n) - 2ull;
            const bool plain = have && ncj != cj && alias == 0 &&
                               (__ballot(idv < Vu) & negs) == negs &&
                               !(kReread && nci == ci && npi != ic);

            bool valid[MAXN + 1];
#pragma unroll
            for (int k = 1; k <= MAXN; ++k)
                valid[k] = !plain && k <= n && t[k] != ci && valid_row(t[k]);
            float part[MAXN + 1];
            part[0] = lane_partial(in, pos);
#pragma unroll
            for (int k = 1; k <= MAXN; ++k) part[k] = lane_partial(in, r[k]);
            wave_sum_all(part);
            float fv = 0.0f;
#pragma unroll
            for (int k = 0; k <= MAXN; ++k) fv = lane == k ? part[k] : fv;
            auto f_of = [&](int k) {
                return __int_as_float(__builtin_amdgcn_readlane(__float_as_int(fv), k));
            };
            R work;
#pragma unroll
            for (int e = 0; e < VEC; ++e) work.v[e] = 0.0f;
            uint64_t act = 0;
            if (plain) {
                const bool skip = fv <= -(float)kMaxExp || fv >= (float)kMaxExp;
                int b = (int)(((double)fv + 6.0) * 83.0);
                b = (uint32_t)b < (uint32_t)kExpTableSize ? b : 0;
                act = __ballot(!skip) & ((2ull << n) - 1ull);
                fv = (((lane == 0 ? 1.0f : 0.0f) - s_exp[b]) * a.lr) * a.alpha;
            }
            auto g_of = f_of;
            float gpos = 0.0f;
            {
                float sig = 0.0f;
                if (plain ? (act & 1ull) != 0 : sigmoid_tab(s_exp, f_of(0), &sig)) {
                    const float g = plain ? g_of(0) : ((1.0f - sig) * a.lr) * a.alpha;
#pragma unroll
                    for (int e = 0; e < VEC; ++e) {
                        work.v[e] = __builtin_fmaf(g, pos.v[e], work.v[e]);
                        pos.v[e] = __builtin_fmaf(g, in.v[e], pos.v[e]);
                    }
                    pos_upd = true;
                    gpos = g;
                    ++nupd;
                }
            }
            bool upd[MAXN + 1];
            float gk[MAXN + 1];
#pragma unroll
            for (int k = 1; k <= MAXN; ++k) {
                upd[k] = false;
                gk[k] = 0.0f;
                float g;
                if (plain) {
                    if (!((act >> k) & 1ull)) continue;
                    g = g_of(k);
                } else {
                    if (!valid[k]) continue;
                    float f = f_of(k);
                    int prev = -1;
#pragma unroll
                    for (int q = 1; q < k; ++q)
                        if (valid[q] && t[q] == t[k]) prev = q;
                    if (prev >= 0) {
#pragma unroll
                        for (int q = 1; q < k; ++q) {
                            if (q == prev) {
                                r[k] = r[q];
                                f = upd[q] ? uniformf(wave_sum(lane_partial(in, r[k]))) : f_of(q);
                            }
                        }
                        fv = lane == k ? f : fv;
                    }
                    float sig;
                    if (!sigmoid_tab(s_exp, f, &sig)) continue;
                    g = ((0.0f - sig) * a.lr) * a.alpha;
                }
#pragma unroll
                for (int e = 0; e < VEC; ++e) {
                    work.v[e] = __builtin_fmaf(g, r[k].v[e], work.v[e]);
                    r[k].v[e] = __builtin_fmaf(g, in.v[e], r[k].v[e]);
                }
                upd[k] = true;
                gk[k] = g;
                ++nupd;
            }
            if (kReread) __builtin_amdgcn_s_waitcnt(kWaitVm0);
#pragma unroll
            for (int k = 1; k <= MAXN; ++k) {
                if (!upd[k]) continue;
                if ((thm >> k) & 1u) {
                    R dlt;
#pragma unroll
                    for (int e = 0; e < VEC; ++e) dlt.v[e] = gk[k] * in.v[e];
                    dlt.atomic_add(a.ctx + (int64_t)t[k] * d, lane, d);
                } else {
                    r[k].store(a.ctx + (int64_t)t[k] * d, lane, d);
                }
                if (!kReread && !plain) {
#pragma unroll
                    for (int q = 1; q <= MAXN; ++q)
                        if (next_target(q) == t[k])
#pragma unroll
                            for (int e = 0; e < VEC; ++e)
                                rn[q].v[e] = __builtin_fmaf(gk[k], in.v[e], rn[q].v[e]);
                    if (have && nci == t[k] && (npi != ic || nhi))
#pragma unroll
                        for (int e = 0; e < VEC; ++e)
                            pos_n.v[e] = __builtin_fmaf(gk[k], in.v[e], pos_n.v[e]);
                }
            }
            padd_on = false;
            if (hot_ci && gpos != 0.0f) {
                R pdl;
#pragma unroll
                for (int e = 0; e < VEC; ++e) pdl.v[e] = gpos * in.v[e];
                pdl.atomic_add(a.ctx + (int64_t)ci * d, lane, d);
                if (kReread) {
                    padd = pdl;
                    padd_on = plain && nci == ci;
                } else {
                    if (!plain)
#pragma unroll
                        for (int q = 1; q <= MAXN; ++q)
                            if (next_target(q) == ci)
#pragma unroll
                                for (int e = 0; e < VEC; ++e) rn[q].v[e] += pdl.v[e];
                    if (have && nci == ci)
#pragma unroll
                        for (int e = 0; e < VEC; ++e) pos_n.v[e] += pdl.v[e];
                }
            } else if (!hot_ci && pos_upd && (!have || npi != ic)) {
                pos.store(a.ctx + (int64_t)ci * d, lane, d);
                if (!kReread) {
                    if (!plain)
#pragma unroll
                        for (int q = 1; q <= MAXN; ++q)
                            if (next_target(q) == ci) rn[q] = pos;
                    if (have && nci == ci) pos_n = pos;
                }
            }
            if (hot_cj) {
                work.atomic_add(a.node + (int64_t)cj * d, lane, d);
            } else {
#pragma unroll
                for (int e = 0; e < VEC; ++e) in.v[e] = in.v[e] + work.v[e];
                in.store(a.node + (int64_t)cj * d, lane, d);
            }
            if (kReread) {
                if (!plain && have) {
                    __builtin_amdgcn_s_waitcnt(kWaitVm0);
                    reread(npi != ic || nhi);
                    __builtin_amdgcn_s_waitcnt(kWaitVm0);
                }
            } else if (have && ncj == cj) {
#pragma unroll
                for (int e = 0; e < VEC; ++e) in_n.v[e] += work.v[e];
            }
        }
        if (a.upd_count && lane == 0 && nupd) atomicAdd(a.upd_count, (unsigned long long)nupd);
    }
}

struct O1Args {
    float *node;
    const int32_t *edges;
    const uint64_t *seeds;
    const uint32_t *table;
    int64_t V;
    int64_t E;
    int d;
    int negative;
    float lr;
    FastMod fm;
    int packed;
    const uint32_t *hot;
    int64_t chunk;
};

template <int VEC, bool FULL, int MAXN>
__global__ void __launch_bounds__(256) k_sgns_o1(O1Args a) {
    using R = Row<VEC, FULL>;
    const int lane = threadIdx.x & 63;
    const int64_t waves_per_block = blockDim.x >> 6;
    const int64_t gw = (int64_t)blockIdx.x * waves_per_block + (threadIdx.x >> 6);
    const int64_t nwaves = (int64_t)gridDim.x * waves_per_block;
    const LcgLane lc = lcg_lane_constants(lane);
    const int n = a.negative;
    const int d = a.d;

    for (int64_t e = gw; e < a.E; e += nwaves) {
        const int u = uniform(a.edges[2 * e]);
        const int v = uniform(a.edges[2 * e + 1]);
        if (u < 0 || u >= a.V || v < 0 || v >= a.V) continue;
        DrawBatch db;
        db.used = 0;
        db.base = uniform64(a.seeds[e]);
        db.target = 0;
        if (n > 0) draws_fill(db, db.base, lc, a, 2 * n);

        int t1[MAXN + 1], t2[MAXN + 1];
        bool v1[MAXN + 1], v2[MAXN + 1];
        t1[0] = v;
        t2[0] = u;
        v1[0] = v2[0] = true;
#pragma unroll
        for (int k = 1; k <= MAXN; ++k) {
            if (k <= n) {
                t1[k] = (int)readlane_u32(db.target, k - 1);
                t2[k] = (int)readlane_u32(db.target, n + k - 1);
                v1[k] = t1[k] != v && t1[k] >= 0 && t1[k] < a.V;
                v2[k] = t2[k] != u && t2[k] >= 0 && t2[k] < a.V;
            } else {
                t1[k] = t2[k] = -1;
                v1[k] = v2[k] = false;
            }
        }
        R in1, in2;
        in1.load(a.node + (int64_t)u * d, lane, d);
        if (v != u) in2.load(a.node + (int64_t)v * d, lane, d);
        const bool hot_u = is_hot(a, u), hot_v = is_hot(a, v);
        R r1[MAXN + 1], r2[MAXN + 1];
#pragma unroll
        for (int k = 1; k <= MAXN; ++k) {
            if (v1[k]) r1[k].load(a.node + (int64_t)t1[k] * d, lane, d);
            if (v2[k]) r2[k].load(a.node + (int64_t)t2[k] * d, lane, d);
        }
        if (v != u) r1[0] = in2; else r1[0] = in1;

        {
            float part[MAXN + 1];
#pragma unroll
            for (int k = 0; k <= MAXN; ++k) part[k] = v1[k] ? lane_partial(in1, r1[k]) : 0.0f;
            wave_sum_n(part, n + 1);
            R work;
#pragma unroll
            for (int q = 0; q < VEC; ++q) work.v[q] = 0.0f;
#pragma unroll
            for (int k = 0; k <= MAXN; ++k) {
                if (!v1[k]) continue;
                float sig;
                if (!sigmoid_ref(uniformf(part[k]), &sig)) continue;
                const float g = ((k == 0 ? 1.0f : 0.0f) - sig) * a.lr;
#pragma unroll
                for (int q = 0; q < VEC; ++q) work.v[q] = __builtin_fmaf(g, r1[k].v[q], work.v[q]);
            }
#pragma unroll
            for (int q = 0; q < VEC; ++q) in1.v[q] = in1.v[q] + work.v[q];
            if (hot_u) work.atomic_add(a.node + (int64_t)u * d, lane, d);
            else in1.store(a.node + (int64_t)u * d, lane, d);
        }
        r2[0] = in1;
        if (v == u) in2 = in1;
        {
            float part[MAXN + 1];
#pragma unroll
            for (int k = 0; k <= MAXN; ++k) part[k] = v2[k] ? lane_partial(in2, r2[k]) : 0.0f;
            wave_sum_n(part, n + 1);
            R work;
#pragma unroll
            for (int q = 0; q < VEC; ++q) work.v[q] = 0.0f;
#pragma unroll
            for (int k = 0; k <= MAXN; ++k) {
                if (!v2[k]) continue;
                float sig;
                if (!sigmoid_ref(uniformf(part[k]), &sig)) continue;
                const float g = ((k == 0 ? 1.0f : 0.0f) - sig) * a.lr;
#pragma unroll
                for (int q = 0; q < VEC; ++q) work.v[q] = __builtin_fmaf(g, r2[k].v[q], work.v[q]);
            }
#pragma unroll
            for (int q = 0; q < VEC; ++q) in2.v[q] = in2.v[q] + work.v[q];
            if (hot_v) work.atomic_add(a.node + (int64_t)v * d, lane, d);
            else in2.store(a.node + (int64_t)v * d, lane, d);
        }
    }
}

template <int VEC, int MAXN>
constexpr int o1_runs_waves_per_eu() {
    return (VEC <= 2 && MAXN <= 5) ? 8 : 1;
}

template <int VEC, bool FULL, int MAXN>
__global__ void __launch_bounds__(256)
    __attribute__((amdgpu_waves_per_eu(o1_runs_waves_per_eu<VEC, MAXN>())))
    k_sgns_o1_runs(O1Args a) {
    using R = Row<VEC, FULL>;
    const int lane = threadIdx.x & 63;
    const int64_t waves_per_block = blockDim.x >> 6;
    const int64_t gw = (int64_t)blockIdx.x * waves_per_block + (threadIdx.x >> 6);
    const int64_t nwaves = (int64_t)gridDim.x * waves_per_block;
    const LcgLane lc = lcg_lane_constants(lane);
    const int n = a.negative;
    const int d = a.d;
    const int64_t nchunks = (a.E + a.chunk - 1) / a.chunk;

    for (int64_t c = gw; c < nchunks; c += nwaves) {
        const int64_t e0 = c * a.chunk;
        const int64_t e1 = e0 + a.chunk < a.E ? e0 + a.chunk : a.E;
        int cu = -1;
        bool hot_cu = false;
        R hu, du;
        auto flush = [&]() {
            if (cu < 0) return;
            if (hot_cu) du.atomic_add(a.node + (int64_t)cu * d, lane, d);
            else hu.store(a.node + (int64_t)cu * d, lane, d);
        };
        for (int64_t e = e0; e < e1; ++e) {
            const int u = uniform(a.edges[2 * e]);
            const int v = uniform(a.edges[2 * e + 1]);
            if (u < 0 || u >= a.V || v < 0 || v >= a.V) continue;
            if (u != cu) {
                flush();
                cu = u;
                hot_cu = is_hot(a, u);
                hu.load(a.node + (int64_t)u * d, lane, d);
#pragma unroll
                for (int q = 0; q < VEC; ++q) du.v[q] = 0.0f;
            }
            DrawBatch db;
            db.used = 0;
            db.base = uniform64(a.seeds[e]);
            db.target = 0;
            if (n > 0) draws_fill(db, db.base, lc, a, 2 * n);
            int t1[MAXN + 1], t2[MAXN + 1];
            bool v1[MAXN + 1], v2[MAXN + 1];
            t1[0] = v;
            t2[0] = u;
            v1[0] = v2[0] = true;
#pragma unroll
            for (int k = 1; k <= MAXN; ++k) {
                if (k <= n) {
                    t1[k] = (int)readlane_u32(db.target, k - 1);
                    t2[k] = (int)readlane_u32(db.target, n + k - 1);
                    v1[k] = t1[k] != v && t1[k] >= 0 && t1[k] < a.V;
                    v2[k] = t2[k] != u && t2[k] >= 0 && t2[k] < a.V;
                } else {
                    t1[k] = t2[k] = -1;
                    v1[k] = v2[k] = false;
                }
            }
            R in2;
            if (v != u) in2.load(a.node + (int64_t)v * d, lane, d);
            const bool hot_v = is_hot(a, v);
            R r1[MAXN + 1], r2[MAXN + 1];
#pragma unroll
            for (int k = 1; k <= MAXN; ++k) {
                if (v1[k]) {
                    if (t1[k] == u) r1[k] = hu;
                    else r1[k].load(a.node + (int64_t)t1[k] * d, lane, d);
                }
                if (v2[k] && t2[k] != v) r2[k].load(a.node + (int64_t)t2[k] * d, lane, d);
            }
            r1[0] = v != u ? in2 : hu;
            {
                float part[MAXN + 1];
#pragma unroll
                for (int k = 0; k <= MAXN; ++k) part[k] = v1[k] ? lane_partial(hu, r1[k]) : 0.0f;
                wave_sum_n(part, n + 1);
                R work;
#pragma unroll
                for (int q = 0; q < VEC; ++q) work.v[q] = 0.0f;
#pragma unroll
                for (int k = 0; k <= MAXN; ++k) {
                    if (!v1[k]) continue;
                    float sig;
                    if (!sigmoid_ref(uniformf(part[k]), &sig)) continue;
                    const float g = ((k == 0 ? 1.0f : 0.0f) - sig) * a.lr;
#pragma unroll
                    for (int q = 0; q < VEC; ++q) work.v[q] = __builtin_fmaf(g, r1[k].v[q], work.v[q]);
                }
#pragma unroll
                for (int q = 0; q < VEC; ++q) {
                    hu.v[q] = hu.v[q] + work.v[q];
                    du.v[q] = du.v[q] + work.v[q];
                }
            }
            r2[0] = hu;
            if (v == u) in2 = hu;
#pragma unroll
            for (int k = 1; k <= MAXN; ++k)
                if (v2[k] && t2[k] == v) r2[k] = in2;
            {
                float part[MAXN + 1];
#pragma unroll
                for (int k = 0; k <= MAXN; ++k) part[k] = v2[k] ? lane_partial(in2, r2[k]) : 0.0f;
                wave_sum_n(part, n + 1);
                R work;
#pragma unroll
                for (int q = 0; q < VEC; ++q) work.v[q] = 0.0f;
#pragma unroll
                for (int k = 0; k <= MAXN; ++k) {
                    if (!v2[k]) continue;
                    float sig;
                    if (!sigmoid_ref(uniformf(part[k]), &sig)) continue;
                    const float g = ((k == 0 ? 1.0f : 0.0f) - sig) * a.lr;
#pragma unroll
                    for (int q = 0; q < VEC; ++q) work.v[q] = __builtin_fmaf(g, r2[k].v[q], work.v[q]);
                }
                if (v == u) {
                    if (hot_cu) flush();
#pragma unroll
                    for (int q = 0; q < VEC; ++q) {
                        hu.v[q] = hu.v[q] + work.v[q];
                        du.v[q] = hot_cu ? work.v[q] : du.v[q] + work.v[q];
                    }
                } else {
#pragma unroll
                    for (int q = 0; q < VEC; ++q) in2.v[q] = in2.v[q] + work.v[q];
                    if (hot_v) work.atomic_add(a.node + (int64_t)v * d, lane, d);
                    else in2.store(a.node + (int64_t)v * d, lane, d);
                }
            }
        }
        flush();
    }
}

struct KernelSet {
    void *o2_direct[2][3];
    void *o2_ring[2][3];
    void *o2_stream[2][3];
    void *o1[2][3];
    void *o1_runs[2][3];
};
#define COME_DECLARE_VEC(V) \
    const KernelSet &kernels_vec##V(); \
    hipError_t upload_exp_table_vec##V(const float *host1000);
COME_DECLARE_VEC(1)
COME_DECLARE_VEC(2)
COME_DECLARE_VEC(4)
COME_DECLARE_VEC(8)
#undef COME_DECLARE_VEC

}
```

### nodeembedding-to-communityembedding_amd/csrc/come_sgns_vec1.hip

```cpp
#include "come_sgns_impl.h"

namespace come {

const KernelSet &kernels_vec1() {
    static KernelSet ks = [] {
        KernelSet k{};
        k.o2_direct[0][0] = (void *)&k_sgns_o2<1, false, 5>;
        k.o1[0][0] = (void *)&k_sgns_o1<1, false, 5>;
        k.o1_runs[0][0] = (void *)&k_sgns_o1_runs<1, false, 5>;
        k.o2_ring[0][0] = (void *)&k_sgns_o2_ring<1, false, 5>;
        k.o2_stream[0][0] = (void *)&k_sgns_o2_stream<1, false, 5>;
        k.o2_direct[0][1] = (void *)&k_sgns_o2<1, false, 10>;
        k.o1[0][1] = (void *)&k_sgns_o1<1, false, 10>;
        k.o1_runs[0][1] = (void *)&k_sgns_o1_runs<1, false, 10>;
        k.o2_ring[0][1] = (void *)&k_sgns_o2_ring<1, false, 10>;
        k.o2_stream[0][1] = (void *)&k_sgns_o2_stream<1, false, 10>;
        k.o2_direct[0][2] = (void *)&k_sgns_o2<1, false, 20>;
        k.o1[0][2] = (void *)&k_sgns_o1<1, false, 20>;
        k.o1_runs[0][2] = (void *)&k_sgns_o1_runs<1, false, 20>;
        k.o2_ring[0][2] = (void *)&k_sgns_o2_ring<1, false, 20>;
        k.o2_stream[0][2] = (void *)&k_sgns_o2_stream<1, false, 20>;
        return k;
    }();
    return ks;
}

hipError_t upload_exp_table_vec1(const float *host1000) {
    return hipMemcpyToSymbol(HIP_SYMBOL(c_exp_table), host1000, sizeof(float) * kExpTableSize);
}

}
```

### nodeembedding-to-communityembedding_amd/csrc/come_sgns_vec2.hip

```cpp
#include "come_sgns_impl.h"

namespace come {

const KernelSet &kernels_vec2() {
    static KernelSet ks = [] {
        KernelSet k{};
        k.o2_direct[0][0] = (void *)&k_sgns_o2<2, false, 5>;
        k.o1[0][0] = (void *)&k_sgns_o1<2, false, 5>;
        k.o1_runs[0][0] = (void *)&k_sgns_o1_runs<2, false, 5>;
        k.o2_ring[0][0] = (void *)&k_sgns_o2_ring<2, false, 5>;
        k.o2_stream[0][0] = (void *)&k_sgns_o2_stream<2, false, 5>;
        k.o2_direct[0][1] = (void *)&k_sgns_o2<2, false, 10>;
        k.o1[0][1] = (void *)&k_sgns_o1<2, false, 10>;
        k.o1_runs[0][1] = (void *)&k_sgns_o1_runs<2, false, 10>;
        k.o2_ring[0][1] = (void *)&k_sgns_o2_ring<2, false, 10>;
        k.o2_stream[0][1] = (void *)&k_sgns_o2_stream<2, false, 10>;
        k.o2_direct[0][2] = (void *)&k_sgns_o2<2, false, 20>;
        k.o1[0][2] = (void *)&k_sgns_o1<2, false, 20>;
        k.o1_runs[0][2] = (void *)&k_sgns_o1_runs<2, false, 20>;
        k.o2_ring[0][2] = (void *)&k_sgns_o2_ring<2, false, 20>;
        k.o2_stream[0][2] = (void *)&k_sgns_o2_stream<2, false, 20>;
        k.o2_direct[1][0] = (void *)&k_sgns_o2<2, true, 5>;
        k.o1[1][0] = (void *)&k_sgns_o1<2, true, 5>;
        k.o1_runs[1][0] = (void *)&k_sgns_o1_runs<2, true, 5>;
        k.o2_ring[1][0] = (void *)&k_sgns_o2_ring<2, true, 5>;
        k.o2_stream[1][0] = (void *)&k_sgns_o2_stream<2, true, 5>;
        k.o2_direct[1][1] = (void *)&k_sgns_o2<2, true, 10>;
        k.o1[1][1] = (void *)&k_sgns_o1<2, true, 10>;
        k.o1_runs[1][1] = (void *)&k_sgns_o1_runs<2, true, 10>;
        k.o2_ring[1][1] = (void *)&k_sgns_o2_ring<2, true, 10>;
        k.o2_stream[1][1] = (void *)&k_sgns_o2_stream<2, true, 10>;
        k.o2_direct[1][2] = (void *)&k_sgns_o2<2, true, 20>;
        k.o1[1][2] = (void *)&k_sgns_o1<2, true, 20>;
        k.o1_runs[1][2] = (void *)&k_sgns_o1_runs<2, true, 20>;
        k.o2_ring[1][2] = (void *)&k_sgns_o2_ring<2, true, 20>;
        k.o2_stream[1][2] = (void *)&k_sgns_o2_stream<2, true, 20>;
        return k;
    }();
    return ks;
}

hipError_t upload_exp_table_vec2(const float *host1000) {
    return hipMemcpyToSymbol(HIP_SYMBOL(c_exp_table), host1000, sizeof(float) * kExpTableSize);
}

}
```

### nodeembedding-to-communityembedding_amd/model.py

```python
import logging as log

import numpy as np

from . import _lib
from .embedding import Vocab
from .io_utils import load_ground_true


class Model(object):
    def __init__(self, nodes_degree, size=2, down_sampling=0, seed=1, table_size=100000000,
                 path_labels='data/', input_file=None, k=None, device=None):
        self.down_sampling = down_sampling
        self.seed = seed
        self.table_size = int(table_size)
        if size % 4 != 0:
            log.warning("consider setting layer size to a multiple of 4 for greater performance")
        self.layer1_size = int(size)
        self.device = device
        if nodes_degree is None:
            raise Exception("Model not initialized, need the nodes degree")
        self.build_vocab_(nodes_degree)
        if k is not None:
            self.ground_true, self.k = None, int(k)
        else:
            self.ground_true, self.k = load_ground_true(path=path_labels, file_name=input_file)
        self.reset_weights()
        self.make_table()

    def build_vocab_(self, vocab):
        if isinstance(vocab, dict):
            ids = np.fromiter(vocab.keys(), np.int64, len(vocab))
            counts = np.fromiter(vocab.values(), np.float64, len(vocab))
        else:
            ids, counts = (np.asarray(vocab[0], np.int64), np.asarray(vocab[1], np.float64))
        order = np.argsort(ids, kind="stable")
        self.node_ids = ids[order]
        self.counts = counts[order]
        assert self.node_ids.min() == 1
        self.vocab_size = len(self.node_ids)
        self._contiguous = bool(self.node_ids[-1] == self.vocab_size)
        self._vocab = None
        self._hot_cache = {}
        self.precalc_sampling()

    def precalc_sampling(self):
        if self.down_sampling:
            total = self.counts.sum()
            thr = float(self.down_sampling) * total
            prob = (np.sqrt(self.counts / thr) + 1) * (thr / self.counts)
            self._sample_prob = np.minimum(prob, 1.0)
        else:
            self._sample_prob = np.ones(self.vocab_size)

    def sample_probability_rows(self):
        return self._sample_prob

    @property
    def vocab(self):
        if self._vocab is None:
            self._vocab = {}
            for i, (nid, c) in enumerate(zip(self.node_ids.tolist(), self.counts.tolist())):
                self._vocab[nid] = Vocab(count=c, index=i, sample_probability=self._sample_prob[i])
        return self._vocab

    def rows_of(self, ids):
        ids = np.asarray(ids, np.int64)
        if self._contiguous:
            r = ids - 1
            r[(ids < 1) | (ids > self.vocab_size)] = -1
            return r
        pos = np.searchsorted(self.node_ids, ids)
        pos_c = np.minimum(pos, self.vocab_size - 1)
        return np.where(self.node_ids[pos_c] == ids, pos_c, -1)

    def _torch_device(self):
        import torch
        if self.device is not None:
            return torch.device(self.device)
        return torch.device("cuda", torch.cuda.current_device()) if torch.cuda.is_available() \
            else torch.device("cpu")

    def reset_weights(self):
        import torch
        dev = self._torch_device()
        V, d, K = self.vocab_size, self.layer1_size, self.k
        node = np.empty((V, d), np.float32)
        step = max(1, (1 << 22) // max(1, d))
        for r0 in range(0, V, step):
            r1 = min(V, r0 + step)
            node[r0:r1] = np.random.uniform(low=-1, high=1, size=(r1 - r0, d))
        self.node_embedding = torch.from_numpy(node).to(dev)
        self.context_embedding = torch.zeros((V, d), dtype=torch.float32, device=dev)
        self.centroid = torch.zeros((K, d), dtype=torch.float32, device=dev)
        self.covariance_mat = torch.zeros((K, d, d), dtype=torch.float32, device=dev)
        self.inv_covariance_mat = torch.zeros((K, d, d), dtype=torch.float32, device=dev)
        self.pi = torch.zeros((V, K), dtype=torch.float32, device=dev)

    def make_table(self, power=0.75):
        import torch
        log.info("constructing a table with noise distribution from %i words" % self.vocab_size)
        c = np.zeros(self.vocab_size + 1, np.float64)
        c[1:] = self.counts
        if not self._contiguous:
            c = np.zeros(self.vocab_size + 1, np.float64)
            ids = self.node_ids
            m = ids <= self.vocab_size
            c[ids[m]] = self.counts[m]
        table = np.zeros(self.table_size, np.uint32)
        _lib.check(_lib.lib().come_make_table(_lib.ptr(c), self.vocab_size, _lib.ptr(table),
                                             self.table_size, float(power)), "come_make_table")
        self.table_host = table
        self.table = torch.from_numpy(table.view(np.int32)).to(self._torch_device())
        self._hot_cache = {}
        self.table_packed = None
        if self.table.is_cuda:
            from .training_sdg_inner import pack_table
            self.table_packed = pack_table(self.table)

    def hot_rows(self, share=None):
        from . import training_sdg_inner as tsi
        share = tsi.default_hot_share(self.layer1_size) if share is None else float(share)
        if not getattr(self.table, "is_cuda", False) or share <= 0:
            return None
        cache = self.__dict__.setdefault("_hot_cache", {})
        key = (share, self.table.data_ptr(), int(self.vocab_size), int(self.table.numel()))
        if key not in cache:
            cache[key] = tsi.hot_rows(self.table, self.vocab_size,
                                      max(1, int(share * self.table.numel())))
        return cache[key]

    def negative_table(self):
        if getattr(self, "use_packed_table", True) and \
                getattr(self, "table_packed", None) is not None:
            return self.table_packed
        return self.table

    def save(self, path='data', file_name=None):
        import os
        import torch
        os.makedirs(path, exist_ok=True)
        state = {}
        for k, v in self.__dict__.items():
            if k in ("_vocab", "table_packed", "_hot_cache"):
                continue
            if isinstance(v, np.ndarray):
                state["np:" + k] = torch.from_numpy(v.view(np.int32) if v.dtype == np.uint32
                                                    else v)
            elif isinstance(v, torch.Tensor):
                state[k] = v.detach().cpu()
            else:
                state[k] = v
        torch.save(state, os.path.join(path, file_name + '.bin'))

    @staticmethod
    def load_model(path='data', file_name=None, device=None):
        import os
        import torch
        state = torch.load(os.path.join(path, file_name + '.bin'), weights_only=True,
                           map_location="cpu")
        m = Model.__new__(Model)
        for k, v in state.items():
            if k.startswith("np:"):
                arr = v.numpy()
                if k == "np:table_host":
                    arr = arr.view(np.uint32)
                setattr(m, k[3:], arr)
            else:
                setattr(m, k, v)
        m._vocab = None
        if device is not None:
            m.device = device
        dev = m._torch_device()
        for k in ("node_embedding", "context_embedding", "centroid", "covariance_mat",
                  "inv_covariance_mat", "pi", "table"):
            setattr(m, k, getattr(m, k).to(dev))
        m.table_packed = None
        if m.table.is_cuda:
            from .training_sdg_inner import pack_table
            m.table_packed = pack_table(m.table)
        log.info('model loaded, size: %d table_size: %d down_sampling: %.5f communities %d' %
                 (m.layer1_size, m.table_size, m.down_sampling, m.k))
        return m
```

### nodeembedding-to-communityembedding_amd/training_sdg_inner.py

```python
import ctypes
import threading

import numpy as np

from . import _lib
from ._lib import (HOT_NONE, MODE_HOGWILD, MODE_SEQUENTIAL, TABLE_PACKED, check, ptr,
                   stream_handle)

FAST_VERSION = 0
MAX_SENTENCE_LEN = 10000
_SEED_LOCK = threading.Lock()


def init():
    return _lib.lib().come_fast_version()


def exp_table():
    out = np.zeros(1000, np.float32)
    _lib.lib().come_exp_table(ptr(out))
    return out


def draw_seeds(n, out=None):
    n = int(n)
    if n == 0:
        return np.zeros(0, np.uint64)
    if out is not None and (out.dtype != np.uint64 or out.shape != (n,) or
                            not out.flags["C_CONTIGUOUS"]):
        raise ValueError("out must be a contiguous uint64 array of %d seeds" % n)
    with _SEED_LOCK:
        st = np.random.get_state()
        if st[0] != "MT19937":
            ab = np.random.randint(0, 2 ** 24, size=2 * n).astype(np.uint64)
            return (ab[0::2] << np.uint64(24)) + ab[1::2]
        state = np.empty(625, np.uint32)
        state[:624] = st[1]
        state[624] = st[2]
        out = np.empty(n, np.uint64) if out is None else out
        check(_lib.lib().come_np_draw_seeds(ptr(state), n, ptr(out)), "come_np_draw_seeds")
        np.random.set_state((st[0], state[:624].copy(), int(state[624]), st[3], st[4]))
    return out


def _require_cuda(t, name, dtype):
    import torch
    if not isinstance(t, torch.Tensor) or not t.is_cuda:
        raise TypeError("%s must be a CUDA tensor" % name)
    if t.dtype != dtype:
        raise TypeError("%s must be %s (got %s)" % (name, dtype, t.dtype))
    if not t.is_contiguous():
        raise ValueError("%s must be contiguous" % name)


class PackedTable(object):

    def __init__(self, words, T):
        self.words, self.T = words, int(T)


def pack_table(table):
    import torch
    _require_cuda(table, "table", torch.int32)
    T = table.numel()
    words = torch.empty(((T + 63) // 64, 4), dtype=torch.int32, device=table.device)
    status = torch.empty(1, dtype=torch.int32, device=table.device)
    check(_lib.lib().come_pack_table(ptr(table), T, ptr(words), ptr(status),
                                     stream_handle(table.device)), "come_pack_table")
    return PackedTable(words, T) if int(status.item()) == 0 else None


def _table_args(table):
    import torch
    if isinstance(table, PackedTable):
        return ptr(table.words), table.T, TABLE_PACKED
    _require_cuda(table, "table", torch.int32)
    return ptr(table), table.numel(), 0


def _opts_arg(opts, update_count=None):
    import ctypes
    if opts is None and update_count is None:
        return None
    if update_count is not None:
        import torch
        _require_cuda(update_count, "update_count", torch.int64)
    o = _lib.launch_opts(update_count, **(opts or {}))
    return ctypes.byref(o)


DEFAULT_HOT_P = 5e-6
DEFAULT_HOT_P_WIDE = 8e-7


def default_hot_share(d):
    return DEFAULT_HOT_P if int(d) <= 128 else DEFAULT_HOT_P_WIDE


def hot_rows(table, V, min_count):
    import torch
    _require_cuda(table, "table", torch.int32)
    counts = torch.empty(int(V), dtype=torch.int32, device=table.device)
    bits = torch.empty((int(V) + 31) // 32, dtype=torch.int32, device=table.device)
    check(_lib.lib().come_hot_rows(ptr(table), table.numel(), int(V), int(min_count), ptr(counts),
                                   ptr(bits), stream_handle(table.device)), "come_hot_rows")
    return bits


def _hot_arg(hot, node, V):
    import torch
    if isinstance(hot, str):
        if hot != "auto":
            raise ValueError("hot must be a bitmap tensor, None or 'auto'")
        return None, 0
    if hot is None:
        return None, HOT_NONE
    _require_cuda(hot, "hot", torch.int32)
    if hot.device != node.device:
        raise ValueError("hot must be on the tables' device (%s, got %s)" % (node.device,
                                                                            hot.device))
    if hot.numel() < (int(V) + 31) // 32:
        raise ValueError("hot bitmap has %d words, needs ceil(V/32) = %d" % (
            hot.numel(), (int(V) + 31) // 32))
    return ptr(hot), 0


def sgns_o2(node, ctx, walks, seeds, window, negative, table, lr, alpha=1.0, mode=MODE_HOGWILD,
            opts=None, update_count=None, hot="auto"):
    import torch
    _require_cuda(node, "node", torch.float32)
    _require_cuda(ctx, "ctx", torch.float32)
    _require_cuda(walks, "walks", torch.int32)
    _require_cuda(seeds, "seeds", torch.int64)
    tp, T, flag = _table_args(table)
    if node.shape != ctx.shape or node.dim() != 2:
        raise ValueError("node and ctx must both be [V, d]")
    if walks.dim() != 2 or seeds.shape != (walks.shape[0],):
        raise ValueError("walks must be [P, L] and seeds [P]")
    if walks.shape[1] > MAX_SENTENCE_LEN:
        walks = walks[:, :MAX_SENTENCE_LEN].contiguous()
    V, d = node.shape
    hp, hflag = _hot_arg(hot, node, V)
    rc = _lib.lib().come_sgns_o2_ex(ptr(node), ptr(ctx), V, d, ptr(walks), walks.shape[0],
                                    walks.shape[1], ptr(seeds), int(window), int(negative),
                                    tp, T, float(lr), float(alpha), int(mode) | flag | hflag,
                                    hp, _opts_arg(opts, update_count),
                                    stream_handle(node.device))
    check(rc, "come_sgns_o2")


def sgns_o1(node, edges, seeds, negative, table, lr, mode=MODE_HOGWILD, opts=None, hot="auto"):
    import torch
    _require_cuda(node, "node", torch.float32)
    _require_cuda(edges, "edges", torch.int32)
    _require_cuda(seeds, "seeds", torch.int64)
    tp, T, flag = _table_args(table)
    if edges.dim() != 2 or edges.shape[1] != 2 or seeds.shape != (edges.shape[0],):
        raise ValueError("edges must be [E, 2] and seeds [E]")
    V, d = node.shape
    hp, hflag = _hot_arg(hot, node, V)
    rc = _lib.lib().come_sgns_o1_ex(ptr(node), V, d, ptr(edges), edges.shape[0], ptr(seeds),
                                    int(negative), tp, T, float(lr), int(mode) | flag | hflag,
                                    hp, _opts_arg(opts), stream_handle(node.device))
    check(rc, "come_sgns_o1")


def sgns_o2_loss(node, ctx, walks, seeds, window, negative, table, return_walks=False):
    import torch
    _require_cuda(node, "node", torch.float32)
    _require_cuda(ctx, "ctx", torch.float32)
    _require_cuda(walks, "walks", torch.int32)
    _require_cuda(seeds, "seeds", torch.int64)
    tp, T, flag = (None, 0, 0) if table is None else _table_args(table)
    if node.shape != ctx.shape or node.dim() != 2:
        raise ValueError("node and ctx must both be [V, d]")
    if walks.dim() != 2 or seeds.shape != (walks.shape[0],):
        raise ValueError("walks must be [P, L] and seeds [P]")
    if walks.shape[1] > MAX_SENTENCE_LEN:
        walks = walks[:, :MAX_SENTENCE_LEN].contiguous()
    V, d = node.shape
    P = walks.shape[0]
    per_walk = torch.zeros(P, dtype=torch.float64, device=node.device) if return_walks else None
    if P:
        out = torch.zeros(2, dtype=torch.float64, device=node.device)
        rc = _lib.lib().come_sgns_o2_loss(
            ptr(node), ptr(ctx), V, d, ptr(walks), P, walks.shape[1], ptr(seeds), int(window),
            int(negative), tp, T, flag, ptr(per_walk) if return_walks else None, ptr(out),
            ptr(out.view(torch.int64)[1:]), stream_handle(node.device))
        check(rc, "come_sgns_o2_loss")
        total, pairs = float(out[0].item()), int(out.view(torch.int64)[1].item())
    else:
        total, pairs = 0.0, 0
    return (total, pairs, per_walk) if return_walks else (total, pairs)


def sgns_pairs_loss(inp, out, rows_in, rows_pos, rows_neg=None, return_pairs=False):
    import torch
    _require_cuda(inp, "inp", torch.float32)
    _require_cuda(out, "out", torch.float32)
    _require_cuda(rows_in, "rows_in", torch.int32)
    _require_cuda(rows_pos, "rows_pos", torch.int32)
    if inp.shape != out.shape or inp.dim() != 2:
        raise ValueError("inp and out must both be [V, d]")
    M = rows_in.shape[0]
    if rows_in.dim() != 1 or rows_pos.shape != (M,):
        raise ValueError("rows_in and rows_pos must both be [M]")
    n = 0
    if rows_neg is not None:
        _require_cuda(rows_neg, "rows_neg", torch.int32)
        if rows_neg.dim() != 2 or rows_neg.shape[0] != M:
            raise ValueError("rows_neg must be [M, n]")
        n = rows_neg.shape[1]
    V, d = inp.shape
    per_pair = torch.zeros(M, dtype=torch.float64, device=inp.device) if return_pairs else None
    if M:
        res = torch.zeros(2, dtype=torch.float64, device=inp.device)
        rc = _lib.lib().come_sgns_pairs_loss(
            ptr(inp), ptr(out), V, d, ptr(rows_in), ptr(rows_pos), ptr(rows_neg) if n else None,
            M, n, ptr(per_pair) if return_pairs else None, ptr(res),
            ptr(res.view(torch.int64)[1:]), stream_handle(inp.device))
        check(rc, "come_sgns_pairs_loss")
        total, counted = float(res[0].item()), int(res.view(torch.int64)[1].item())
    else:
        total, counted = 0.0, 0
    return (total, counted, per_pair) if return_pairs else (total, counted)


def count_o2_pairs(walks_np, window):
    w = np.ascontiguousarray(walks_np, np.int32)
    if w.ndim != 2 or w.size == 0:
        return 0
    return int(_lib.lib().come_count_o2_pairs(ptr(w), w.shape[0], w.shape[1], int(window)))



_DEVICE_LOCK = threading.Lock()
_NUMPY_ROUTE = ["host"]


def set_numpy_route(route):
    if route not in ("host", "device"):
        raise ValueError("route must be 'host' or 'device'")
    prev, _NUMPY_ROUTE[0] = _NUMPY_ROUTE[0], route
    return prev


_PYEXT = []


def _pyext():
    if _PYEXT:
        return _PYEXT[0]
    with _SEED_LOCK:
        if not _PYEXT:
            try:
                from . import _come_pyext as ext
            except ImportError as e:
                raise _lib.ComeError("_come_pyext is not built (%s): run `make -C "
                                     "nodeembedding-to-communityembedding_amd/csrc`" % e)
            L = _lib.lib()
            addr = lambda f: ctypes.cast(f, ctypes.c_void_p).value
            ext.init(addr(L.come_cpu_sgns_o2), addr(L.come_cpu_sgns_o1), addr(L.come_last_error),
                     np.random.randint)
            _PYEXT.append(ext)
    return _PYEXT[0]


def _call_seed():
    return (1 << 24) * int(np.random.randint(0, 1 << 24)) + int(np.random.randint(0, 1 << 24))


def _rows_of(items):
    return np.array([-1 if it is None else int(it.index) for it in items], np.int32)


def _host_table_arg(arr, name):
    if not (isinstance(arr, np.ndarray) and arr.dtype == np.float32 and arr.ndim == 2 and
            arr.flags.c_contiguous and arr.flags.writeable):
        raise TypeError("%s must be a writable C-contiguous float32 [V, d] numpy array or a CUDA "
                        "tensor" % name)
    return arr


def _host_neg_table(table):
    t = np.asarray(table)
    if t.dtype == np.int32:
        t = t.view(np.uint32)
    if t.dtype != np.uint32 or not t.flags.c_contiguous:
        t = np.ascontiguousarray(t, np.uint32)
    return t


class _Mirrors(object):

    def __init__(self):
        self.tables = {}
        self.neg = {}

    def table(self, arr, device):
        import torch
        key = (arr.__array_interface__["data"][0], arr.shape, arr.dtype.str, str(device))
        t = self.tables.get(key)
        if t is None:
            if len(self.tables) >= 16:
                self.tables.clear()
            t = self.tables[key] = torch.empty(arr.shape, dtype=torch.float32, device=device)
        return t

    @staticmethod
    def _fingerprint(arr):
        idx = np.linspace(0, len(arr) - 1, 64).astype(np.int64)
        return arr[idx].tobytes()

    def negative_table(self, arr, device):
        import torch
        key = (arr.__array_interface__["data"][0], arr.shape[0], str(device))
        fp = self._fingerprint(arr)
        hit = self.neg.get(key)
        if hit is None or hit[0] != fp:
            if len(self.neg) >= 4:
                self.neg.clear()
            hit = self.neg[key] = (fp, torch.from_numpy(arr.view(np.int32)).to(device))
        return hit[1]


_MIRRORS = _Mirrors()


def _device_of(*arrays):
    import torch
    for a in arrays:
        if isinstance(a, torch.Tensor):
            if not a.is_cuda:
                raise TypeError("tables must be CUDA tensors or numpy arrays")
            return a.device
    return torch.device("cuda", torch.cuda.current_device())


def _is_tensor(a):
    import torch
    return isinstance(a, torch.Tensor)


def _resolve_table(py_table, device):
    import torch
    if isinstance(py_table, torch.Tensor):
        t = py_table if py_table.dtype == torch.int32 else py_table.view(torch.int32)
        return t.to(device), None
    host = _host_neg_table(py_table)
    return _MIRRORS.negative_table(host, device), host


def _draw_rows(seed, count, host_table):
    out = np.empty(int(count), np.uint32)
    if count:
        check(_lib.lib().come_lcg_table_draws(int(seed), int(count), ptr(host_table),
                                              host_table.shape[0], ptr(out)),
              "come_lcg_table_draws")
    return out.astype(np.int64)


class _Borrowed(object):

    def __init__(self, arr, device, rows):
        import torch
        self.arr = arr
        if isinstance(arr, torch.Tensor):
            self.dev, self.rows = arr, None
            return
        _host_table_arg(arr, "embedding table")
        self.dev = _MIRRORS.table(arr, device)
        r = np.unique(rows)
        self.rows = r[(r >= 0) & (r < arr.shape[0])]
        if len(self.rows):
            ri = torch.from_numpy(self.rows).to(device)
            self.ridx = ri
            self.dev.index_copy_(0, ri, torch.from_numpy(arr[self.rows]).to(device))

    def writeback(self):
        if self.rows is not None and len(self.rows):
            self.arr[self.rows] = self.dev.index_select(0, self.ridx).cpu().numpy()


def _host_o2(node, ctx, rows, nr, lr, negative, window, table, alpha):
    _host_table_arg(node, "py_node_embedding")
    _host_table_arg(ctx, "py_context_embedding")
    if node.shape != ctx.shape:
        raise ValueError("node and context embeddings must have the same shape")
    tab = _host_neg_table(table)
    seed = ctypes.c_uint64(nr)
    check(_lib.lib().come_cpu_sgns_o2(node.ctypes.data, ctx.ctypes.data, node.shape[0],
                                      node.shape[1], rows.ctypes.data, 1, rows.shape[0],
                                      ctypes.byref(seed), int(window), int(negative),
                                      tab.ctypes.data, tab.shape[0], float(lr), float(alpha),
                                      MODE_SEQUENTIAL, 1, None), "come_cpu_sgns_o2")


def _device_o2(node_in, ctx_in, rows, nr, lr, negative, window, table_in, alpha):
    import torch
    device = _device_of(node_in, ctx_in, table_in)
    table, host_table = _resolve_table(table_in, device)
    walk_rows = rows[rows >= 0].astype(np.int64)
    ctx_rows = walk_rows
    if not _is_tensor(ctx_in):
        if host_table is None:
            host_table = table.cpu().numpy().view(np.uint32)
        pairs = count_o2_pairs(rows.reshape(1, -1), window)
        ctx_rows = np.concatenate([walk_rows, _draw_rows(nr, pairs * int(negative),
                                                         host_table)])
    node = _Borrowed(node_in, device, walk_rows)
    ctx = _Borrowed(ctx_in, device, ctx_rows)
    walks = torch.from_numpy(rows.reshape(1, -1)).to(device)
    seeds = torch.from_numpy(np.array([nr], np.uint64).view(np.int64)).to(device)
    sgns_o2(node.dev, ctx.dev, walks, seeds, window, negative, table, lr, alpha, MODE_SEQUENTIAL)
    node.writeback()
    ctx.writeback()


def _route(*args):
    tensors = [_is_tensor(a) for a in args]
    if all(tensors):
        return "device"
    if any(tensors) or _NUMPY_ROUTE[0] == "device":
        return "locked"
    return "host"


def train_o2(py_node_embedding, py_context_embedding, py_path, py_lr, py_negative, py_window,
             py_table, py_alpha=1.0, py_size=None, py_work=None):
    if (type(py_node_embedding) is np.ndarray and type(py_context_embedding) is np.ndarray and
            type(py_table) is np.ndarray and _NUMPY_ROUTE[0] == "host"):
        try:
            return _pyext().train_o2(py_node_embedding, py_context_embedding, py_path, py_lr,
                                     py_negative, py_window, py_table, py_alpha)
        except TypeError:
            pass
    nr = _call_seed()
    rows = _rows_of(py_path[:MAX_SENTENCE_LEN] if isinstance(py_path, (list, tuple))
                    else list(py_path)[:MAX_SENTENCE_LEN])
    result = int((rows >= 0).sum())
    if not rows.size:
        return result
    args = (py_node_embedding, py_context_embedding, rows, nr, py_lr, py_negative, py_window,
            py_table, py_alpha)
    route = _route(py_node_embedding, py_context_embedding, py_table)
    if route == "host":
        _host_o2(*args)
    elif route == "device":
        _device_o2(*args)
    else:
        with _DEVICE_LOCK:
            _device_o2(*args)
    return result


def _host_o1(node, rows, nr, lr, negative, table):
    _host_table_arg(node, "py_node_embedding")
    tab = _host_neg_table(table)
    seed = ctypes.c_uint64(nr)
    check(_lib.lib().come_cpu_sgns_o1(node.ctypes.data, node.shape[0], node.shape[1],
                                      rows.ctypes.data, 1, ctypes.byref(seed), int(negative),
                                      tab.ctypes.data, tab.shape[0], float(lr), MODE_SEQUENTIAL,
                                      1, None), "come_cpu_sgns_o1")


def _device_o1(node_in, rows, nr, lr, negative, table_in):
    import torch
    device = _device_of(node_in, table_in)
    table, host_table = _resolve_table(table_in, device)
    touched = rows[rows >= 0].astype(np.int64)
    if not _is_tensor(node_in):
        if host_table is None:
            host_table = table.cpu().numpy().view(np.uint32)
        touched = np.concatenate([touched, _draw_rows(nr, 2 * int(negative), host_table)])
    node = _Borrowed(node_in, device, touched)
    edges = torch.from_numpy(rows.reshape(1, 2)).to(device)
    seeds = torch.from_numpy(np.array([nr], np.uint64).view(np.int64)).to(device)
    sgns_o1(node.dev, edges, seeds, negative, table, lr, MODE_SEQUENTIAL)
    node.writeback()


def train_o1(py_node_embedding, py_edge, py_lr, py_negative, py_table, py_size=None, py_work=None):
    if (type(py_node_embedding) is np.ndarray and type(py_table) is np.ndarray and
            _NUMPY_ROUTE[0] == "host"):
        try:
            return _pyext().train_o1(py_node_embedding, py_edge, py_lr, py_negative, py_table)
        except TypeError:
            pass
    nr = _call_seed()
    rows = _rows_of(list(py_edge)[:2])
    result = int((rows >= 0).sum())
    if rows.size != 2:
        return result
    args = (py_node_embedding, rows, nr, py_lr, py_negative, py_table)
    route = _route(py_node_embedding, py_table)
    if route == "host":
        _host_o1(*args)
    elif route == "device":
        _device_o1(*args)
    else:
        with _DEVICE_LOCK:
            _device_o1(*args)
    return result
```

Baseline: 1.125 billion.

## Cache quiet node rows in an LDS window ring in the streaming SGNS kernel

```diff
diff --git a/include/come.h b/include/come.h
--- a/include/come.h
+++ b/include/come.h
@@ -189,6 +189,14 @@
 
 int come_hot_rows(const uint32_t *table, uint64_t T, int64_t V, uint64_t min_count,
                   uint32_t *counts, uint32_t *hot_bits, void *stream);
+int come_quiet_rows(const uint32_t *table, uint64_t T, int64_t V, double power, int id_shift,
+                    double visitors, double eps, uint64_t hot_min_count, uint32_t *counts,
+                    double *sum, uint32_t *quiet_bits, void *stream);
+int come_sgns_o2_quiet(float *node, float *ctx, int64_t V, int d, const int32_t *walks, int64_t P,
+                       int L, const uint64_t *seeds, int window, int negative,
+                       const uint32_t *table, uint64_t T, float lr, float alpha, int mode,
+                       const uint32_t *hot_rows, const uint32_t *quiet_rows,
+                       const come_launch_opts *opts, void *stream);
 int come_sgns_o1_ex(float *node, int64_t V, int d, const int32_t *edges, int64_t E,
                     const uint64_t *seeds, int negative, const uint32_t *table, uint64_t T,
                     float lr, int mode, const uint32_t *hot_rows, const come_launch_opts *opts,
diff --git a/nodeembedding-to-communityembedding_amd/_lib.py b/nodeembedding-to-communityembedding_amd/_lib.py
--- a/nodeembedding-to-communityembedding_amd/_lib.py
+++ b/nodeembedding-to-communityembedding_amd/_lib.py
@@ -30,7 +30,8 @@
            "come_community_loss", "come_cpu_community_loss", "come_sgns_o2_loss",
            "come_sgns_pairs_loss", "come_cpu_sgns_o2_loss", "come_cpu_sgns_pairs_loss",
            "come_gmm_estep_diag", "come_gmm_diag_scratch", "come_gmm_diag_moments",
-           "come_gmm_diag_scatter", "come_community_grad_diag", "come_community_loss_diag")
+           "come_gmm_diag_scatter", "come_community_grad_diag", "come_community_loss_diag",
+           "come_quiet_rows", "come_sgns_o2_quiet")
 
 OPTION_FIELDS = ("o2_kernel", "o2_blocks_per_cu", "o2_waves_per_block",
                  "o2_static", "rows_per_wave", "o1_rows_per_wave",
@@ -120,6 +121,9 @@
     L.come_sgns_o2_ex.argtypes = [P, P, i64, i32, P, i64, i32, P, i32, i32, P, u64, f32, f32, i32,
                                   P, P, P]
     L.come_hot_rows.argtypes = [P, u64, i64, u64, P, P, P]
+    L.come_quiet_rows.argtypes = [P, u64, i64, f64, i32, f64, f64, u64, P, P, P, P]
+    L.come_sgns_o2_quiet.argtypes = [P, P, i64, i32, P, i64, i32, P, i32, i32, P, u64, f32, f32,
+                                     i32, P, P, P, P]
     L.come_lcg_table_draws.argtypes = [u64, i64, P, u64, P]
     L.come_delta_flags.argtypes = [P, P, i64, i32, P, P]
     L.come_delta_gather.argtypes = [P, P, P, i64, i32, P, P, P]
diff --git a/nodeembedding-to-communityembedding_amd/context_embeddings.py b/nodeembedding-to-communityembedding_amd/context_embeddings.py
--- a/nodeembedding-to-communityembedding_amd/context_embeddings.py
+++ b/nodeembedding-to-communityembedding_amd/context_embeddings.py
@@ -22,7 +22,7 @@
     def __init__(self, lr=0.1, window_size=5, workers=1, negative=5, deterministic=False,
                  batch_walks=1 << 20, distributed=False, sync_walks=DEFAULT_SYNC_WALKS,
                  sparse_sync=False, overlap=True, group=None, hot_share=None, launch_opts=None,
-                 combine="touched_mean"):
+                 combine="touched_mean", quiet_eps=None):
         self.lr = float(lr)
         self.workers = workers
         self.negative = negative
@@ -36,6 +36,7 @@
         self.group = group
         self.hot_share = hot_share
         self.launch_opts = launch_opts
+        self.quiet_eps = quiet_eps
         self.combine = combine
         self._exchanges = {}
         if self.distributed and self.deterministic:
@@ -129,12 +130,30 @@
                  elapsed, pairs / elapsed if elapsed else 0.0)
         return pairs
 
+    def quiet_rows(self, model, walks):
+        import torch
+        eps = tsi.DEFAULT_QUIET_EPS if self.quiet_eps is None else float(self.quiet_eps)
+        dev = model.node_embedding.device
+        if eps <= 0 or dev.type != "cuda" or self.window_size > 5 or self.negative > 5 \
+                or model.layer1_size > 128:
+            return None
+        opts = self.launch_opts or {}
+        bpc = int(opts.get("o2_blocks_per_cu", 0)) or tsi.QUIET_BLOCKS_PER_CU
+        waves = 4 * bpc * torch.cuda.get_device_properties(dev).multi_processor_count
+        if int(opts.get("max_waves", 0)) > 0:
+            waves = min(waves, int(opts["max_waves"]))
+        waves = max(1, min(waves, int(walks), self.batch_walks))
+        if int(opts.get("o2_kernel", 0)) != 3 and model.vocab_size < 32 * waves:
+            return None
+        return model.quiet_rows(waves, self.window_size, eps, self.hot_share)
+
     def train_rows(self, model, rows, seeds, alpha=1.0, n_batches=None, update_count=None,
                    launch_events=None):
         import torch
         dev = model.node_embedding.device
         mode = tsi.MODE_SEQUENTIAL if self.deterministic else tsi.MODE_HOGWILD
         hot = None if self.deterministic else model.hot_rows(self.hot_share)
+        quiet = None if self.deterministic else self.quiet_rows(model, rows.shape[0])
         table = model.negative_table()
         rank, world = self.world()
         ex = self.exchange(model) if world > 1 else None
@@ -160,7 +179,8 @@
                     ev[0].record(stream)
                 tsi.sgns_o2(model.node_embedding, model.context_embedding, w, sd,
                             self.window_size, self.negative, table, self.lr, alpha, mode,
-                            opts=self.launch_opts, hot=hot, update_count=update_count)
+                            opts=self.launch_opts, hot=hot, update_count=update_count,
+                            **({} if quiet is None else {"quiet": quiet}))
                 if launch_events is not None:
                     ev[1].record(stream)
                     launch_events.append(ev)
diff --git a/nodeembedding-to-communityembedding_amd/csrc/come_hot.hip b/nodeembedding-to-communityembedding_amd/csrc/come_hot.hip
--- a/nodeembedding-to-communityembedding_amd/csrc/come_hot.hip
+++ b/nodeembedding-to-communityembedding_amd/csrc/come_hot.hip
@@ -62,6 +62,38 @@
     }
 }
 
+
+__global__ void __launch_bounds__(256) k_quiet_sum(const uint32_t *__restrict__ counts, int64_t V,
+                                                   double inv_power, double *__restrict__ sum) {
+    double s = 0.0;
+    for (int64_t v = (int64_t)blockIdx.x * blockDim.x + threadIdx.x; v < V;
+         v += (int64_t)gridDim.x * blockDim.x)
+        s += pow((double)counts[v], inv_power);
+    for (int o = 32; o > 0; o >>= 1) s += __shfl_down(s, o);
+    if ((threadIdx.x & 63) == 0 && s != 0.0) atomicAdd(sum, s);
+}
+
+__global__ void __launch_bounds__(256) k_quiet_bits(const uint32_t *__restrict__ counts, int64_t V,
+                                                    int id_shift, double inv_power,
+                                                    double visitors, double eps,
+                                                    uint64_t hot_min_count,
+                                                    const double *__restrict__ sum,
+                                                    uint32_t *__restrict__ quiet_bits) {
+    const int64_t words = (V + 31) / 32;
+    const double bound = eps * sum[0] / visitors;
+    for (int64_t w = (int64_t)blockIdx.x * blockDim.x + threadIdx.x; w < words;
+         w += (int64_t)gridDim.x * blockDim.x) {
+        uint32_t bits = 0;
+        for (int b = 0; b < 32; ++b) {
+            const int64_t r = 32 * w + b, own = r + id_shift;
+            if (r < V && own >= 0 && own < V && counts[r] < hot_min_count &&
+                pow((double)counts[own], inv_power) <= bound)
+                bits |= 1u << b;
+        }
+        quiet_bits[w] = bits;
+    }
+}
+
 static int hot_rows_impl(int dev, const uint32_t *table, uint64_t T, int packed, int64_t V,
                          uint64_t min_count, uint32_t *counts, uint32_t *hot_bits, void *stream) {
     hipError_t e = hipMemsetAsync(counts, 0, sizeof(uint32_t) * (size_t)V, (hipStream_t)stream);
@@ -113,3 +145,40 @@
     if (rc) return rc;
     return hot_rows_impl(dev, table, T, 0, V, min_count, counts, hot_bits, stream);
 }
+
+extern "C" int come_quiet_rows(const uint32_t *table, uint64_t T, int64_t V, double power,
+                               int id_shift, double visitors, double eps, uint64_t hot_min_count,
+                               uint32_t *counts, double *sum, uint32_t *quiet_bits, void *stream) {
+    if (V <= 0 || V > INT32_MAX) return set_error(COME_E_INVALID, "quiet_rows: V out of range");
+    if (!table || !counts || !sum || !quiet_bits || T == 0)
+        return set_error(COME_E_INVALID, "quiet_rows: null pointer or empty table");
+    if (!(power > 0.0) || !(visitors > 0.0) || !(eps >= 0.0))
+        return set_error(COME_E_INVALID, "quiet_rows: power and visitors must be > 0, eps >= 0");
+    int dev = 0;
+    int rc = ensure_init(&dev);
+    if (rc) return rc;
+    hipError_t e = hipMemsetAsync(counts, 0, sizeof(uint32_t) * (size_t)V, (hipStream_t)stream);
+    if (e != hipSuccess) return hip_error(e, "hipMemsetAsync(counts)");
+    e = hipMemsetAsync(sum, 0, sizeof(double), (hipStream_t)stream);
+    if (e != hipSuccess) return hip_error(e, "hipMemsetAsync(sum)");
+    uint64_t blocks = (T + 255) / 256;
+    const uint64_t cap = (uint64_t)num_cus(dev) * 16;
+    if (blocks > cap) blocks = cap;
+    hipLaunchKernelGGL(k_table_counts, dim3((unsigned)blocks), dim3(256), 0, (hipStream_t)stream,
+                       table, T, V, counts);
+    rc = hip_error(hipGetLastError(), "k_table_counts launch");
+    if (rc) return rc;
+    int64_t vb = (V + 255) / 256;
+    if (vb > 4096) vb = 4096;
+    hipLaunchKernelGGL(k_quiet_sum, dim3((unsigned)vb), dim3(256), 0, (hipStream_t)stream,
+                       (const uint32_t *)counts, V, 1.0 / power, sum);
+    rc = hip_error(hipGetLastError(), "k_quiet_sum launch");
+    if (rc) return rc;
+    const int64_t words = (V + 31) / 32;
+    int64_t wb = (words + 255) / 256;
+    if (wb > 4096) wb = 4096;
+    hipLaunchKernelGGL(k_quiet_bits, dim3((unsigned)wb), dim3(256), 0, (hipStream_t)stream,
+                       (const uint32_t *)counts, V, id_shift, 1.0 / power, visitors, eps,
+                       hot_min_count, (const double *)sum, quiet_bits);
+    return hip_error(hipGetLastError(), "k_quiet_bits launch");
+}
diff --git a/nodeembedding-to-communityembedding_amd/csrc/come_sgns.hip b/nodeembedding-to-communityembedding_amd/csrc/come_sgns.hip
--- a/nodeembedding-to-communityembedding_amd/csrc/come_sgns.hip
+++ b/nodeembedding-to-communityembedding_amd/csrc/come_sgns.hip
@@ -105,11 +105,11 @@
     return ((uintptr_t)p % bytes) == 0;
 }
 
-extern "C" int come_sgns_o2_ex(float *node, float *ctx, int64_t V, int d, const int32_t *walks,
-                               int64_t P, int L, const uint64_t *seeds, int window, int negative,
-                               const uint32_t *table, uint64_t T, float lr, float alpha, int mode,
-                               const uint32_t *hot_rows, const come_launch_opts *opts,
-                               void *stream) {
+static int sgns_o2_impl(float *node, float *ctx, int64_t V, int d, const int32_t *walks,
+                        int64_t P, int L, const uint64_t *seeds, int window, int negative,
+                        const uint32_t *table, uint64_t T, float lr, float alpha, int mode,
+                        const uint32_t *hot_rows, const uint32_t *quiet_rows,
+                        const come_launch_opts *opts, void *stream) {
     const come_launch_opts o = opts ? *opts : current_opts();
     int packed = 0, hot_none = 0;
     int rc = check_common(V, d, negative, table, T, mode, packed, hot_none);
@@ -135,7 +135,7 @@
     O2Args a{node, ctx, walks, seeds, table, V, P, L, d, window, negative, lr, alpha,
              make_fastmod(T), packed, nullptr,
              reinterpret_cast<unsigned long long *>(o.o2_update_count), o.o2_fresh_loads,
-             o.o2_atomic_writeback, mode == COME_MODE_HOGWILD ? hot_rows : nullptr};
+             o.o2_atomic_writeback, mode == COME_MODE_HOGWILD ? hot_rows : nullptr, nullptr};
     int full = 0;
     const KernelSet &ks = kernel_set(d, &full);
     const int mi = maxn_index(negative);
@@ -145,14 +145,18 @@
         int dev = 0;
         rc = ensure_init(&dev);
         if (rc) return rc;
-        const int bpc = o.o2_blocks_per_cu > 0 ? o.o2_blocks_per_cu : 8;
+        void *win = quiet_rows != nullptr && mi == 0 && window <= kWinMaxW && V < (1ll << 30)
+                        ? ks.o2_stream_win[full] : nullptr;
+        const int bpc = o.o2_blocks_per_cu > 0 ? o.o2_blocks_per_cu : win ? 5 : 8;
         const int64_t hcap = hog_max_blocks(o, V, wpb, o.rows_per_wave);
         int64_t blocks = (P + wpb - 1) / wpb;
         if (blocks > (int64_t)num_cus(dev) * bpc) blocks = (int64_t)num_cus(dev) * bpc;
         if (hcap > 0 && blocks > hcap) blocks = hcap;
         if (o.o2_kernel == 3 || V >= kStreamRowsPerWave * wpb * blocks) {
             if (!o.o2_static) a.counter = launch_counter(dev, stream);
-            return launch(o, ks.o2_stream[full][mi], &a, P, mode, wpb, bpc, 0, stream, hcap);
+            if (win) a.quiet = quiet_rows;
+            return launch(o, win ? win : ks.o2_stream[full][mi], &a, P, mode, wpb, bpc, 0, stream,
+                          hcap);
         }
     }
     const int rs = 2 * window + 1;
@@ -163,6 +167,25 @@
     return launch(o, ks.o2_direct[full][mi], &a, P, mode, wpb,
                   o.o2_blocks_per_cu > 0 ? o.o2_blocks_per_cu : 6, 0, stream,
                   hog ? hog_max_blocks(o, V, wpb, o.rows_per_wave) : 0);
+}
+
+extern "C" int come_sgns_o2_ex(float *node, float *ctx, int64_t V, int d, const int32_t *walks,
+                               int64_t P, int L, const uint64_t *seeds, int window, int negative,
+                               const uint32_t *table, uint64_t T, float lr, float alpha, int mode,
+                               const uint32_t *hot_rows, const come_launch_opts *opts,
+                               void *stream) {
+    return sgns_o2_impl(node, ctx, V, d, walks, P, L, seeds, window, negative, table, T, lr, alpha,
+                        mode, hot_rows, nullptr, opts, stream);
+}
+
+extern "C" int come_sgns_o2_quiet(float *node, float *ctx, int64_t V, int d, const int32_t *walks,
+                                  int64_t P, int L, const uint64_t *seeds, int window,
+                                  int negative, const uint32_t *table, uint64_t T, float lr,
+                                  float alpha, int mode, const uint32_t *hot_rows,
+                                  const uint32_t *quiet_rows, const come_launch_opts *opts,
+                                  void *stream) {
+    return sgns_o2_impl(node, ctx, V, d, walks, P, L, seeds, window, negative, table, T, lr, alpha,
+                        mode, hot_rows, quiet_rows, opts, stream);
 }
 
 extern "C" int come_sgns_o2(float *node, float *ctx, int64_t V, int d, const int32_t *walks,
diff --git a/nodeembedding-to-communityembedding_amd/csrc/come_sgns_impl.h b/nodeembedding-to-communityembedding_amd/csrc/come_sgns_impl.h
--- a/nodeembedding-to-communityembedding_amd/csrc/come_sgns_impl.h
+++ b/nodeembedding-to-communityembedding_amd/csrc/come_sgns_impl.h
@@ -258,6 +258,7 @@
     int fresh;
     int wb_atomic;
     const uint32_t *hot;
+    const uint32_t *quiet;
 };
 
 template <class Args>
@@ -694,15 +695,19 @@
     }
 }
 
-template <int VEC, int MAXN>
+constexpr int kWinMaxW = 5;
+constexpr int kWinSlots = 2 * kWinMaxW + 1;
+
+template <int VEC, int MAXN, bool WINDOW>
 constexpr int stream_waves_per_eu() {
-    return (VEC <= 2 && MAXN <= 5) ? 8 : 1;
-}
-
-template <int VEC, bool FULL, int MAXN>
+    return WINDOW ? 5 : (VEC <= 2 && MAXN <= 5) ? 8 : 1;
+}
+
+template <int VEC, bool FULL, int MAXN, bool WINDOW = false>
 __global__ void __launch_bounds__(256)
-    __attribute__((amdgpu_waves_per_eu(stream_waves_per_eu<VEC, MAXN>())))
+    __attribute__((amdgpu_waves_per_eu(stream_waves_per_eu<VEC, MAXN, WINDOW>())))
     k_sgns_o2_stream(O2Args a) {
+    static_assert(!WINDOW || VEC <= 2, "the window ring holds rows of d <= 128");
     using R = Row<VEC, FULL>;
     const int lane = threadIdx.x & 63;
     const int64_t waves_per_block = blockDim.x >> 6;
@@ -717,6 +722,8 @@
     auto valid_row = [&](int r) { return (uint32_t)r < Vu; };
     constexpr bool kReread = VEC <= 2;
     constexpr uint32_t kHotBit = 0x80000000u;
+    constexpr uint32_t kQuietBit = WINDOW ? 0x40000000u : 0u;
+    constexpr uint32_t kFlagBits = kHotBit | kQuietBit;
     constexpr int kWaitVm0 = 0x0F70;
     __shared__ float s_exp[kExpTableSize];
     for (int i = threadIdx.x; i < kExpTableSize; i += blockDim.x) s_exp[i] = c_exp_table[i];
@@ -725,6 +732,11 @@
     uint32_t *draws = s_draws[threadIdx.x >> 6];
     __shared__ int s_walk[4][128];
     int *wpos = s_walk[threadIdx.x >> 6];
+    float *ring = nullptr;
+    if constexpr (WINDOW) {
+        __shared__ float s_ring[4][kWinSlots * 64 * VEC];
+        ring = s_ring[threadIdx.x >> 6];
+    }
 
     for (int64_t p = a.counter ? next_unit(a.counter, 0, 0, lane) : gw; p < a.P;
          p = next_unit(a.counter, p, nwaves, lane)) {
@@ -735,6 +747,9 @@
             if (!valid_row(v)) return -1;
             if (a.hot != nullptr && ((a.hot[(uint32_t)v >> 5] >> (v & 31)) & 1u))
                 v = (int)((uint32_t)v | kHotBit);
+            else if (WINDOW && a.quiet != nullptr &&
+                     ((a.quiet[(uint32_t)v >> 5] >> (v & 31)) & 1u))
+                v = (int)((uint32_t)v | kQuietBit);
             return v;
         };
         int wbase = 0;
@@ -752,6 +767,7 @@
             return uniform(wpos[q - wbase]);
         };
         int it_i = 0, it_j = -1;
+        bool nqj = false;
         auto next_pair = [&](int &ci, int &cj, int &pi, bool &hi, bool &hj) -> bool {
             for (;;) {
                 if (it_i >= path_len) return false;
@@ -769,8 +785,9 @@
                 if (j == i) continue;
                 const int rcj = raw_at(j);
                 if (rcj == -1) continue;
-                ci = (int)((uint32_t)rci & ~kHotBit);
-                cj = (int)((uint32_t)rcj & ~kHotBit);
+                ci = (int)((uint32_t)rci & ~kFlagBits);
+                cj = (int)((uint32_t)rcj & ~kFlagBits);
+                if constexpr (WINDOW) nqj = ((uint32_t)rcj & kQuietBit) != 0;
                 hi = ((uint32_t)rci & kHotBit) != 0;
                 hj = ((uint32_t)rcj & kHotBit) != 0;
                 pi = i;
@@ -809,8 +826,23 @@
         auto next_target = [&](int k) {
             return k <= n ? (int)(readlane_u32(ids, 32 + k) & ~kHotBit) : -1;
         };
+        int ring_ids = -1;
+        auto ring_find = [&](int id) {
+            const uint64_t m = __ballot(ring_ids == id);
+            return m ? (int)__builtin_ctzll(m) : -1;
+        };
+        auto ring_write_back = [&](int s) {
+            const int id = (int)readlane_u32((uint32_t)ring_ids, s);
+            R out;
+#pragma unroll
+            for (int e = 0; e < VEC; ++e) out.v[e] = ring[(s * VEC + e) * 64 + lane];
+            out.store(a.node + (int64_t)id * d, lane, d);
+            ring_ids = lane == s ? -1 : ring_ids;
+        };
         auto prefetch = [&](bool need_pos) {
-            in_n.load(a.node + (int64_t)ncj * d, lane, d);
+            bool held = false;
+            if constexpr (WINDOW) held = nqj && ring_find(ncj) >= 0;
+            if (!held) in_n.load(a.node + (int64_t)ncj * d, lane, d);
             if (need_pos) pos_n.load(a.ctx + (int64_t)nci * d, lane, d);
             const bool drawn = lane > 32 && lane <= 32 + n;
             const uint32_t nx = drawn ? draws[drawn ? dp.used + lane - 33 : 0] : 0xFFFFFFFFu;
@@ -840,6 +872,7 @@
         while (have) {
             const int ci = nci, cj = ncj, ic = npi;
             const bool hot_ci = nhi, hot_cj = nhj;
+            const bool quiet_cj = WINDOW && nqj;
             R in = in_n;
             int t[MAXN + 1];
             R r[MAXN + 1];
@@ -857,6 +890,31 @@
             }
             if (new_center) pos_upd = false;
             prev_i = ic;
+            int slot = -1;
+            if constexpr (WINDOW) {
+                uint64_t occ = new_center ? __ballot(ring_ids >= 0) : 0;
+                if (occ) {
+                    (void)raw_at(ic + w < path_len ? ic + w : path_len - 1);
+                    const int q = ic - w + lane;
+                    int wid = -1;
+                    if (lane <= 2 * w && q >= 0 && q < path_len) {
+                        const int v = wpos[q - wbase];
+                        wid = v == -1 ? -1 : (int)((uint32_t)v & ~kFlagBits);
+                    }
+                    while (occ) {
+                        const int s = __builtin_ctzll(occ);
+                        occ &= occ - 1;
+                        const int id = (int)readlane_u32((uint32_t)ring_ids, s);
+                        if (__ballot(wid == id) == 0) ring_write_back(s);
+                    }
+                }
+                if (quiet_cj) {
+                    slot = ring_find(cj);
+                    if (slot >= 0)
+#pragma unroll
+                        for (int e = 0; e < VEC; ++e) in.v[e] = ring[(slot * VEC + e) * 64 + lane];
+                }
+            }
             ids = (uint32_t)__builtin_amdgcn_permlane32_swap((int)ids, (int)ids, false, false)[1];
             const uint32_t thm = (uint32_t)__ballot((ids & kHotBit) != 0);
             advance();
@@ -1015,7 +1073,22 @@
             } else {
 #pragma unroll
                 for (int e = 0; e < VEC; ++e) in.v[e] = in.v[e] + work.v[e];
-                in.store(a.node + (int64_t)cj * d, lane, d);
+                bool to_ring = false;
+                if constexpr (WINDOW) {
+                    if (quiet_cj && slot < 0) {
+                        const uint64_t free_slots =
+                            ~__ballot(ring_ids >= 0) & ((1ull << kWinSlots) - 1ull);
+                        if (free_slots) {
+                            slot = __builtin_ctzll(free_slots);
+                            ring_ids = lane == slot ? cj : ring_ids;
+                        }
+                    }
+                    to_ring = quiet_cj && slot >= 0;
+                    if (to_ring)
+#pragma unroll
+                        for (int e = 0; e < VEC; ++e) ring[(slot * VEC + e) * 64 + lane] = in.v[e];
+                }
+                if (!to_ring) in.store(a.node + (int64_t)cj * d, lane, d);
             }
             if (kReread) {
                 if (!plain && have) {
@@ -1026,6 +1099,14 @@
             } else if (have && ncj == cj) {
 #pragma unroll
                 for (int e = 0; e < VEC; ++e) in_n.v[e] += work.v[e];
+            }
+        }
+        if constexpr (WINDOW) {
+            uint64_t occ = __ballot(ring_ids >= 0);
+            while (occ) {
+                const int s = __builtin_ctzll(occ);
+                occ &= occ - 1;
+                ring_write_back(s);
             }
         }
         if (a.upd_count && lane == 0 && nupd) atomicAdd(a.upd_count, (unsigned long long)nupd);
@@ -1292,6 +1373,7 @@
     void *o2_direct[2][3];
     void *o2_ring[2][3];
     void *o2_stream[2][3];
+    void *o2_stream_win[2];
     void *o1[2][3];
     void *o1_runs[2][3];
 };
diff --git a/nodeembedding-to-communityembedding_amd/csrc/come_sgns_vec1.hip b/nodeembedding-to-communityembedding_amd/csrc/come_sgns_vec1.hip
--- a/nodeembedding-to-communityembedding_amd/csrc/come_sgns_vec1.hip
+++ b/nodeembedding-to-communityembedding_amd/csrc/come_sgns_vec1.hip
@@ -20,6 +20,7 @@
         k.o1_runs[0][2] = (void *)&k_sgns_o1_runs<1, false, 20>;
         k.o2_ring[0][2] = (void *)&k_sgns_o2_ring<1, false, 20>;
         k.o2_stream[0][2] = (void *)&k_sgns_o2_stream<1, false, 20>;
+        k.o2_stream_win[0] = (void *)&k_sgns_o2_stream<1, false, 5, true>;
         return k;
     }();
     return ks;
diff --git a/nodeembedding-to-communityembedding_amd/csrc/come_sgns_vec2.hip b/nodeembedding-to-communityembedding_amd/csrc/come_sgns_vec2.hip
--- a/nodeembedding-to-communityembedding_amd/csrc/come_sgns_vec2.hip
+++ b/nodeembedding-to-communityembedding_amd/csrc/come_sgns_vec2.hip
@@ -35,6 +35,8 @@
         k.o1_runs[1][2] = (void *)&k_sgns_o1_runs<2, true, 20>;
         k.o2_ring[1][2] = (void *)&k_sgns_o2_ring<2, true, 20>;
         k.o2_stream[1][2] = (void *)&k_sgns_o2_stream<2, true, 20>;
+        k.o2_stream_win[0] = (void *)&k_sgns_o2_stream<2, false, 5, true>;
+        k.o2_stream_win[1] = (void *)&k_sgns_o2_stream<2, true, 5, true>;
         return k;
     }();
     return ks;
diff --git a/nodeembedding-to-communityembedding_amd/model.py b/nodeembedding-to-communityembedding_amd/model.py
--- a/nodeembedding-to-communityembedding_amd/model.py
+++ b/nodeembedding-to-communityembedding_amd/model.py
@@ -129,6 +129,21 @@
                                       max(1, int(share * self.table.numel())))
         return cache[key]
 
+    def quiet_rows(self, waves, window, eps=None, hot_share=None):
+        from . import training_sdg_inner as tsi
+        eps = tsi.DEFAULT_QUIET_EPS if eps is None else float(eps)
+        share = tsi.default_hot_share(self.layer1_size) if hot_share is None else float(hot_share)
+        if not getattr(self.table, "is_cuda", False) or eps <= 0 or not self._contiguous:
+            return None
+        T = int(self.table.numel())
+        visitors = float(waves) * (2 * int(window) + 1)
+        hot_min = max(1, int(share * T)) if share > 0 else T + 1
+        cache = self.__dict__.setdefault("_hot_cache", {})
+        key = ("quiet", eps, visitors, hot_min, self.table.data_ptr(), int(self.vocab_size), T)
+        if key not in cache:
+            cache[key] = tsi.quiet_rows(self.table, self.vocab_size, visitors, eps, hot_min)
+        return cache[key]
+
     def negative_table(self):
         if getattr(self, "use_packed_table", True) and \
                 getattr(self, "table_packed", None) is not None:
diff --git a/nodeembedding-to-communityembedding_amd/training_sdg_inner.py b/nodeembedding-to-communityembedding_amd/training_sdg_inner.py
--- a/nodeembedding-to-communityembedding_amd/training_sdg_inner.py
+++ b/nodeembedding-to-communityembedding_amd/training_sdg_inner.py
@@ -107,6 +107,23 @@
     return bits
 
 
+def quiet_rows(table, V, visitors, eps, hot_min_count, power=0.75, id_shift=1):
+    import torch
+    _require_cuda(table, "table", torch.int32)
+    counts = torch.empty(int(V), dtype=torch.int32, device=table.device)
+    total = torch.empty(1, dtype=torch.float64, device=table.device)
+    bits = torch.empty((int(V) + 31) // 32, dtype=torch.int32, device=table.device)
+    check(_lib.lib().come_quiet_rows(ptr(table), table.numel(), int(V), float(power),
+                                     int(id_shift), float(visitors), float(eps),
+                                     int(hot_min_count), ptr(counts), ptr(total), ptr(bits),
+                                     stream_handle(table.device)), "come_quiet_rows")
+    return bits
+
+
+DEFAULT_QUIET_EPS = 0.4
+QUIET_BLOCKS_PER_CU = 5
+
+
 def _hot_arg(hot, node, V):
     import torch
     if isinstance(hot, str):
@@ -126,7 +143,7 @@
 
 
 def sgns_o2(node, ctx, walks, seeds, window, negative, table, lr, alpha=1.0, mode=MODE_HOGWILD,
-            opts=None, update_count=None, hot="auto"):
+            opts=None, update_count=None, hot="auto", quiet=None):
     import torch
     _require_cuda(node, "node", torch.float32)
     _require_cuda(ctx, "ctx", torch.float32)
@@ -141,11 +158,14 @@
         walks = walks[:, :MAX_SENTENCE_LEN].contiguous()
     V, d = node.shape
     hp, hflag = _hot_arg(hot, node, V)
-    rc = _lib.lib().come_sgns_o2_ex(ptr(node), ptr(ctx), V, d, ptr(walks), walks.shape[0],
-                                    walks.shape[1], ptr(seeds), int(window), int(negative),
-                                    tp, T, float(lr), float(alpha), int(mode) | flag | hflag,
-                                    hp, _opts_arg(opts, update_count),
-                                    stream_handle(node.device))
+    qp = None
+    if quiet is not None:
+        qp, _ = _hot_arg(quiet, node, V)
+    rc = _lib.lib().come_sgns_o2_quiet(ptr(node), ptr(ctx), V, d, ptr(walks), walks.shape[0],
+                                       walks.shape[1], ptr(seeds), int(window), int(negative),
+                                       tp, T, float(lr), float(alpha), int(mode) | flag | hflag,
+                                       hp, qp, _opts_arg(opts, update_count),
+                                       stream_handle(node.device))
     check(rc, "come_sgns_o2")
 
 
```

Measured after the change: 1.262 billion, median of 6. +12.1%, better.
